# youngalip/clip-lora-match

Hardware: AMD Instinct MI355X
Metric: image+text embeds/sec & cosine top-k QPS, ViT-B/32+LoRA, 1/2/4/8 MI355X (higher is better)
Workload: dtype bf16 (vision) + fp16 (text); 1 GPU; ViT-B/32 + LoRA r=8 alpha=16 (q,k,v,out, both towers) encode + L2-normalise; per_gpu_batch=256, global_batch=256, seq_len=77, image_size=224, lora_mode=merged, parallelism=dp1

## Files before the change

clip-lora-match_amd/csrc/capi.cpp:

```cpp
#include <hip/hip_runtime.h>

#include <algorithm>
#include <cmath>
#include <map>
#include <mutex>
#include <tuple>
#include <cstdlib>
#include <cstring>
#include <string>
#include <unordered_map>
#include <vector>

#include "clm.h"
#include "kernels.hpp"

using namespace clm;

namespace {

thread_local std::string g_err;
int g_gemm_debug = getenv("CLM_GEMM_DEBUG") ? atoi(getenv("CLM_GEMM_DEBUG")) : 0;
int fail(int code, const std::string& msg) {
  g_err = msg;
  return code;
}
#define HIPCHK(x)                                                                              \
  do {                                                                                         \
    hipError_t e_ = (x);                                                                       \
    if (e_ != hipSuccess) return fail(CLM_E_HIP, std::string(#x) + ": " + hipGetErrorString(e_)); \
  } while (0)

struct DeviceGuard {
  int prev = -1;
  explicit DeviceGuard(int dev) {
    if (hipGetDevice(&prev) != hipSuccess) prev = -1;
    if (prev != dev) (void)hipSetDevice(dev);
  }
  ~DeviceGuard() {
    int cur = -1;
    if (prev >= 0 && hipGetDevice(&cur) == hipSuccess && cur != prev) (void)hipSetDevice(prev);
  }
};

bool is_device_ptr(const void* p) {
  if (!p) return false;
  hipPointerAttribute_t a;
  if (hipPointerGetAttributes(&a, p) != hipSuccess) {
    (void)hipGetLastError();
    return false;
  }
  return a.type == hipMemoryTypeDevice;
}

uint16_t host_f32_to_bf16(float f) {
  uint32_t u;
  std::memcpy(&u, &f, 4);
  if ((u & 0x7fffffffu) > 0x7f800000u) return (uint16_t)((u >> 16) | 0x40);
  u += 0x7fffu + ((u >> 16) & 1u);
  return (uint16_t)(u >> 16);
}
uint16_t host_f32_to_f16(float f) {
  _Float16 h = (_Float16)f;
  uint16_t r;
  std::memcpy(&r, &h, 2);
  return r;
}
float host_f16_to_f32(uint16_t v) {
  _Float16 h;
  std::memcpy(&h, &v, 2);
  return (float)h;
}
float host_bf16_to_f32(uint16_t v) {
  uint32_t u = (uint32_t)v << 16;
  float f;
  std::memcpy(&f, &u, 4);
  return f;
}

int64_t round_up(int64_t x, int64_t m) { return (x + m - 1) / m * m; }

struct HostTensor {
  std::vector<int64_t> shape;
  std::vector<float> data;
};

struct LayerW {
  float *ln1_g = nullptr, *ln1_b = nullptr, *ln2_g = nullptr, *ln2_b = nullptr;
  u16* w_qkv = nullptr; float* b_qkv = nullptr; int k_qkv = 0, kl_qkv = 0;
  u16* w_out = nullptr; float* b_out = nullptr; int k_out = 0, kl_out = 0;
  u16* w_fc1 = nullptr; float* b_fc1 = nullptr; int k_fc1 = 0, kl_fc1 = 0;
  u16* w_fc2 = nullptr; float* b_fc2 = nullptr; int k_fc2 = 0, kl_fc2 = 0;
  u16* a_qkv = nullptr; int r_qkv = 0;
  u16* a_out = nullptr; int r_out = 0;
  u16* a_fc1 = nullptr; int r_fc1 = 0;
  u16* a_fc2 = nullptr; int r_fc2 = 0;
};

struct Tower {
  bool vision = false;
  bool q_log2e = false;
  int d = 0, L = 0, H = 0, mlp = 0;
  std::vector<LayerW> layers;
  float *projT = nullptr, *fin_g = nullptr, *fin_b = nullptr;
  u16* patch_w = nullptr; int kp = 0;
  float *cls = nullptr, *pos = nullptr, *pre_g = nullptr, *pre_b = nullptr, *lut = nullptr;
  float *tok = nullptr, *tpos = nullptr;
  int64_t maxM = 0;
  float* h = nullptr;
  u16 *X = nullptr, *QKV = nullptr, *O = nullptr, *Hm = nullptr, *P = nullptr;
  float* pooled = nullptr;
  float* hc = nullptr;
  u16* Oc = nullptr;
  int *vl_lens = nullptr, *vl_offs = nullptr, *vl_rowmap = nullptr, *vl_tiles = nullptr, *vl_counts = nullptr;
  int64_t ldx = 0, ldo = 0, ldm = 0;
};

constexpr int RPAD = 64;
constexpr int LORA_GRANULE = 32;

}

struct clm_ctx {
  int dev = 0;
  clm_model_desc desc{};
  bool finalized = false;
  bool lora_enabled = true;
  std::unordered_map<std::string, HostTensor> host;
  std::vector<void*> allocs;
  Tower vis, txt;
  void* stage_in = nullptr; size_t stage_in_bytes = 0;
  void* stage_out = nullptr; size_t stage_out_bytes = 0;
  int32_t* ids_dev = nullptr;
  static constexpr int MAX_SPLIT = 4;
  hipStream_t ps[2 * MAX_SPLIT] = {};
  hipEvent_t pev[2 * MAX_SPLIT] = {};
  hipEvent_t ev_fork = nullptr, ev_done = nullptr;
  typedef std::tuple<const void*, int, int, const void*, int, int, void*, void*, int, int, int> PairKey;
  std::map<PairKey, hipGraphExec_t> graphs;
  int last_pair_path = -1;
  bool prof = false;
  std::vector<hipEvent_t> ev_pool;
  size_t ev_used = 0;
  struct Rec { int cat; double work; size_t e0, e1; };
  std::vector<Rec> recs;

  bool bf16(bool vision) const {
    return desc.compute_dtype == CLM_BF16 || (vision && desc.compute_dtype == CLM_COMPUTE_MIXED);
  }

  template <typename T>
  int dalloc(T** p, size_t count) {
    void* q = nullptr;
    if (count == 0) count = 1;
    if (hipMalloc(&q, count * sizeof(T)) != hipSuccess) {
      (void)hipGetLastError();
      return fail(CLM_E_OOM, "hipMalloc of " + std::to_string(count * sizeof(T)) + " bytes failed");
    }
    allocs.push_back(q);
    *p = (T*)q;
    return CLM_OK;
  }
  void drop_graphs() {
    for (auto& kv : graphs) (void)hipGraphExecDestroy(kv.second);
    graphs.clear();
  }
  void free_all() {
    drop_graphs();
    for (void* p : allocs) (void)hipFree(p);
    allocs.clear();
    if (stage_in) (void)hipFree(stage_in);
    if (stage_out) (void)hipFree(stage_out);
    stage_in = stage_out = nullptr;
    stage_in_bytes = stage_out_bytes = 0;
    vis = Tower();
    txt = Tower();
    ids_dev = nullptr;
  }
};

struct clm_index {
  int dev = 0;
  int64_t cap = 0, n = 0, dim = 0, offset = 0;
  u16* rows = nullptr;
  float* inv = nullptr;
  float* rows32 = nullptr;
  void* ws = nullptr; size_t ws_bytes = 0;
  void* ws2 = nullptr; size_t ws2_bytes = 0;
  void* ws3 = nullptr; size_t ws3_bytes = 0;
  void* ws4 = nullptr; size_t ws4_bytes = 0;
  u16* samp = nullptr; float* samp_inv = nullptr; int64_t samp_S = 0, samp_n = -1, samp_cap = 0;
  unsigned* inv_keys = nullptr; int64_t inv_keys_n = -1;
  int64_t search_stats[11] = {0, 0, 0, 0, 0, 0, 0, 0, 0, 0, 0};
};

namespace {

const HostTensor* find(const clm_ctx* c, const std::string& n) {
  auto it = c->host.find(n);
  return it == c->host.end() ? nullptr : &it->second;
}

int need(const clm_ctx* c, const std::string& n, int64_t numel, const HostTensor** out) {
  const HostTensor* t = find(c, n);
  if (!t) return fail(CLM_E_MISSING, "missing tensor '" + n + "'");
  if ((int64_t)t->data.size() != numel)
    return fail(CLM_E_ARG, "tensor '" + n + "' has " + std::to_string(t->data.size()) + " elements, expected " +
                               std::to_string(numel));
  *out = t;
  return CLM_OK;
}

int upload_f32(clm_ctx* c, const std::vector<float>& v, float** dst) {
  int r = c->dalloc(dst, v.size());
  if (r) return r;
  HIPCHK(hipMemcpy(*dst, v.data(), v.size() * sizeof(float), hipMemcpyHostToDevice));
  return CLM_OK;
}

int upload_16(clm_ctx* c, const std::vector<float>& v, u16** dst, bool bf) {
  std::vector<u16> h(v.size());
  if (bf)
    for (size_t i = 0; i < v.size(); ++i) h[i] = host_f32_to_bf16(v[i]);
  else
    for (size_t i = 0; i < v.size(); ++i) h[i] = host_f32_to_f16(v[i]);
  int r = c->dalloc(dst, h.size());
  if (r) return r;
  HIPCHK(hipMemcpy(*dst, h.data(), h.size() * sizeof(u16), hipMemcpyHostToDevice));
  return CLM_OK;
}

int upload_lora_a(clm_ctx* c, const std::vector<float>& A, int r_ext, int in, u16** dst, bool bf) {
  std::vector<float> pad((size_t)RPAD * in, 0.f);
  std::copy(A.begin(), A.begin() + (size_t)r_ext * in, pad.begin());
  return upload_16(c, pad, dst, bf);
}

int get_f32(clm_ctx* c, const std::string& n, int64_t numel, float** dst) {
  const HostTensor* t;
  int r = need(c, n, numel, &t);
  if (r) return r;
  return upload_f32(c, t->data, dst);
}

struct LinearSpec {
  std::string path;
  int in, out;
  bool lora;
};

int build_fused(clm_ctx* c, const std::vector<LinearSpec>& specs, float q_scale, std::vector<float>& W,
                std::vector<float>& bias, int& K, std::vector<float>& A_stack, int& r_ext, int& K_log) {
  const clm_model_desc& d = c->desc;
  const bool unmerged = d.lora_mode == CLM_LORA_UNMERGED;
  const int in = specs[0].in;
  int total_out = 0;
  r_ext = 0;
  for (auto& s : specs) {
    total_out += s.out;
    if (s.lora) r_ext += d.lora_r;
  }
  K = (unmerged && r_ext > 0) ? in + RPAD : in;
  K_log = (unmerged && r_ext > 0) ? in + (r_ext + LORA_GRANULE - 1) / LORA_GRANULE * LORA_GRANULE : in;
  if (r_ext > RPAD) return fail(CLM_E_ARG, "LoRA rank too large for the K-extension (sum r > 64)");
  W.assign((size_t)total_out * K, 0.f);
  bias.assign(total_out, 0.f);
  A_stack.assign((size_t)r_ext * in, 0.f);
  const float scaling = d.lora_r > 0 ? d.lora_alpha / (float)d.lora_r : 0.f;
  int row0 = 0, roff = 0;
  for (size_t si = 0; si < specs.size(); ++si) {
    const LinearSpec& s = specs[si];
    const HostTensor *w, *b;
    int r = need(c, s.path + ".weight", (int64_t)s.out * s.in, &w);
    if (r) return r;
    r = need(c, s.path + ".bias", s.out, &b);
    if (r) return r;
    const float qs = si == 0 ? q_scale : 1.0f;
    for (int o = 0; o < s.out; ++o) {
      std::memcpy(&W[(size_t)(row0 + o) * K], &w->data[(size_t)o * s.in], s.in * sizeof(float));
      bias[row0 + o] = b->data[o];
    }
    if (s.lora) {
      const HostTensor *A, *B;
      const std::string base = "base_model.model." + s.path;
      r = need(c, base + ".lora_A.weight", (int64_t)d.lora_r * s.in, &A);
      if (r) return r;
      r = need(c, base + ".lora_B.weight", (int64_t)s.out * d.lora_r, &B);
      if (r) return r;
      if (!unmerged) {
        for (int o = 0; o < s.out; ++o) {
          float* wr = &W[(size_t)(row0 + o) * K];
          for (int j = 0; j < d.lora_r; ++j) {
            const float bj = scaling * B->data[(size_t)o * d.lora_r + j];
            const float* ar = &A->data[(size_t)j * s.in];
            for (int i = 0; i < s.in; ++i) wr[i] += bj * ar[i];
          }
        }
      } else {
        for (int o = 0; o < s.out; ++o)
          for (int j = 0; j < d.lora_r; ++j)
            W[(size_t)(row0 + o) * K + s.in + roff + j] = scaling * B->data[(size_t)o * d.lora_r + j];
        std::memcpy(&A_stack[(size_t)roff * in], A->data.data(), (size_t)d.lora_r * in * sizeof(float));
      }
      roff += d.lora_r;
    }
    if (qs != 1.0f) {
      for (int o = 0; o < s.out; ++o) {
        float* wr = &W[(size_t)(row0 + o) * K];
        for (int i = 0; i < K; ++i) wr[i] *= qs;
        bias[row0 + o] *= qs;
      }
    }
    row0 += s.out;
  }
  if (!unmerged) r_ext = 0;
  return CLM_OK;
}

int build_tower(clm_ctx* c, Tower& T, bool vision) {
  const clm_model_desc& d = c->desc;
  const clm_tower_desc& td = vision ? d.vision : d.text;
  T.vision = vision;
  T.d = td.hidden; T.L = td.layers; T.H = td.heads; T.mlp = td.mlp;
  if (T.d != T.H * 64) return fail(CLM_E_ARG, "head_dim must be 64");
  if (T.d % 128 || T.d > 1024 || T.mlp % 64) return fail(CLM_E_ARG, "hidden must be a multiple of 128 (<=1024), mlp of 64");
  const std::string pre = vision ? "vision_model" : "text_model";
  const bool lora_on = c->lora_enabled && d.lora_r > 0;
  const uint32_t tg = lora_on ? d.lora_targets : 0u;
  const bool unmerged = d.lora_mode == CLM_LORA_UNMERGED;
  const int Tseq = vision ? (d.image_size / d.patch) * (d.image_size / d.patch) + 1 : 0;
  T.q_log2e = vision && attention_folds_log2e(c->bf16(true), false, Tseq);
  const float qscale = T.q_log2e ? 0.125f * 1.4426950408889634f : 0.125f;
  int r;
  T.layers.resize(T.L);
  for (int l = 0; l < T.L; ++l) {
    LayerW& Lw = T.layers[l];
    const std::string p = pre + ".encoder.layers." + std::to_string(l);
    if ((r = get_f32(c, p + ".layer_norm1.weight", T.d, &Lw.ln1_g))) return r;
    if ((r = get_f32(c, p + ".layer_norm1.bias", T.d, &Lw.ln1_b))) return r;
    if ((r = get_f32(c, p + ".layer_norm2.weight", T.d, &Lw.ln2_g))) return r;
    if ((r = get_f32(c, p + ".layer_norm2.bias", T.d, &Lw.ln2_b))) return r;
    std::vector<float> W, b, A;
    int K, rext, KL;
    std::vector<LinearSpec> qkv = {{p + ".self_attn.q_proj", T.d, T.d, (tg & CLM_LORA_Q) != 0},
                                   {p + ".self_attn.k_proj", T.d, T.d, (tg & CLM_LORA_K) != 0},
                                   {p + ".self_attn.v_proj", T.d, T.d, (tg & CLM_LORA_V) != 0}};
    if ((r = build_fused(c, qkv, qscale, W, b, K, A, rext, KL))) return r;
    if ((r = upload_16(c, W, &Lw.w_qkv, c->bf16(vision))) || (r = upload_f32(c, b, &Lw.b_qkv))) return r;
    Lw.k_qkv = K; Lw.kl_qkv = KL; Lw.r_qkv = rext;
    if (unmerged && rext && (r = upload_lora_a(c, A, rext, T.d, &Lw.a_qkv, c->bf16(vision)))) return r;

    std::vector<LinearSpec> outp = {{p + ".self_attn.out_proj", T.d, T.d, (tg & CLM_LORA_OUT) != 0}};
    if ((r = build_fused(c, outp, 1.0f, W, b, K, A, rext, KL))) return r;
    if ((r = upload_16(c, W, &Lw.w_out, c->bf16(vision))) || (r = upload_f32(c, b, &Lw.b_out))) return r;
    Lw.k_out = K; Lw.kl_out = KL; Lw.r_out = rext;
    if (unmerged && rext && (r = upload_lora_a(c, A, rext, T.d, &Lw.a_out, c->bf16(vision)))) return r;

    std::vector<LinearSpec> fc1 = {{p + ".mlp.fc1", T.d, T.mlp, (tg & CLM_LORA_FC1) != 0}};
    if ((r = build_fused(c, fc1, 1.0f, W, b, K, A, rext, KL))) return r;
    if ((r = upload_16(c, W, &Lw.w_fc1, c->bf16(vision))) || (r = upload_f32(c, b, &Lw.b_fc1))) return r;
    Lw.k_fc1 = K; Lw.kl_fc1 = KL; Lw.r_fc1 = rext;
    if (unmerged && rext && (r = upload_lora_a(c, A, rext, T.d, &Lw.a_fc1, c->bf16(vision)))) return r;

    std::vector<LinearSpec> fc2 = {{p + ".mlp.fc2", T.mlp, T.d, (tg & CLM_LORA_FC2) != 0}};
    if ((r = build_fused(c, fc2, 1.0f, W, b, K, A, rext, KL))) return r;
    if ((r = upload_16(c, W, &Lw.w_fc2, c->bf16(vision))) || (r = upload_f32(c, b, &Lw.b_fc2))) return r;
    Lw.k_fc2 = K; Lw.kl_fc2 = KL; Lw.r_fc2 = rext;
    if (unmerged && rext && (r = upload_lora_a(c, A, rext, T.mlp, &Lw.a_fc2, c->bf16(vision)))) return r;
  }
  {
    const HostTensor* pw;
    const std::string pn = vision ? "visual_projection.weight" : "text_projection.weight";
    if ((r = need(c, pn, (int64_t)d.proj_dim * T.d, &pw))) return r;
    std::vector<float> pt((size_t)T.d * d.proj_dim);
    for (int j = 0; j < d.proj_dim; ++j)
      for (int i = 0; i < T.d; ++i) pt[(size_t)i * d.proj_dim + j] = pw->data[(size_t)j * T.d + i];
    if ((r = upload_f32(c, pt, &T.projT))) return r;
  }
  const int64_t B = d.max_batch;
  if (vision) {
    const int G = d.image_size / d.patch, Tn = G * G + 1;
    if ((r = get_f32(c, pre + ".post_layernorm.weight", T.d, &T.fin_g))) return r;
    if ((r = get_f32(c, pre + ".post_layernorm.bias", T.d, &T.fin_b))) return r;
    if ((r = get_f32(c, pre + ".pre_layrnorm.weight", T.d, &T.pre_g))) return r;
    if ((r = get_f32(c, pre + ".pre_layrnorm.bias", T.d, &T.pre_b))) return r;
    if ((r = get_f32(c, pre + ".embeddings.class_embedding", T.d, &T.cls))) return r;
    if ((r = get_f32(c, pre + ".embeddings.position_embedding.weight", (int64_t)Tn * T.d, &T.pos))) return r;
    const int kreal = d.channels * d.patch * d.patch;
    T.kp = (int)round_up(kreal, 64);
    const HostTensor* pw;
    if ((r = need(c, pre + ".embeddings.patch_embedding.weight", (int64_t)T.d * kreal, &pw))) return r;
    std::vector<float> wp((size_t)T.d * T.kp, 0.f);
    for (int o = 0; o < T.d; ++o) std::memcpy(&wp[(size_t)o * T.kp], &pw->data[(size_t)o * kreal], kreal * 4);
    if ((r = upload_16(c, wp, &T.patch_w, c->bf16(true)))) return r;
    std::vector<float> lut((size_t)d.channels * 256);
    for (int ch = 0; ch < d.channels; ++ch)
      for (int u = 0; u < 256; ++u) {
        const float x = (float)((double)u * (1.0 / 255.0));
        lut[(size_t)ch * 256 + u] = (x - d.mean[ch % 3]) / d.std[ch % 3];
      }
    if ((r = upload_f32(c, lut, &T.lut))) return r;
    T.maxM = B * Tn;
    if ((r = c->dalloc(&T.P, (size_t)B * G * G * T.kp))) return r;
  } else {
    if ((r = get_f32(c, pre + ".final_layer_norm.weight", T.d, &T.fin_g))) return r;
    if ((r = get_f32(c, pre + ".final_layer_norm.bias", T.d, &T.fin_b))) return r;
    if ((r = get_f32(c, pre + ".embeddings.token_embedding.weight", (int64_t)d.vocab * T.d, &T.tok))) return r;
    if ((r = get_f32(c, pre + ".embeddings.position_embedding.weight", (int64_t)d.max_pos * T.d, &T.tpos))) return r;
    T.maxM = B * d.max_pos;
  }
  T.ldx = T.d + RPAD;
  T.ldo = T.d + RPAD;
  T.ldm = T.mlp + RPAD;
  if ((r = c->dalloc(&T.h, (size_t)T.maxM * T.d))) return r;
  if ((r = c->dalloc(&T.X, (size_t)T.maxM * T.ldx))) return r;
  if ((r = c->dalloc(&T.QKV, (size_t)T.maxM * 3 * T.d))) return r;
  if ((r = c->dalloc(&T.O, (size_t)T.maxM * T.ldo))) return r;
  if ((r = c->dalloc(&T.Hm, (size_t)T.maxM * T.ldm))) return r;
  if ((r = c->dalloc(&T.pooled, (size_t)B * d.proj_dim))) return r;
  if ((r = c->dalloc(&T.hc, (size_t)B * T.d))) return r;
  if ((r = c->dalloc(&T.Oc, (size_t)B * T.ldo))) return r;
  if (!T.vision) {
    if ((r = c->dalloc(&T.vl_lens, (size_t)B))) return r;
    if ((r = c->dalloc(&T.vl_offs, (size_t)2 * B + 1))) return r;
    if ((r = c->dalloc(&T.vl_rowmap, (size_t)T.maxM))) return r;
    if ((r = c->dalloc(&T.vl_tiles, (size_t)B))) return r;
    if ((r = c->dalloc(&T.vl_counts, (size_t)2 * B))) return r;
  }
  return CLM_OK;
}

int ensure_stage(void** p, size_t* cap, size_t bytes) {
  if (*cap >= bytes) return CLM_OK;
  if (*p) (void)hipFree(*p);
  *p = nullptr;
  *cap = 0;
  if (hipMalloc(p, bytes) != hipSuccess) {
    (void)hipGetLastError();
    *p = nullptr;
    return fail(CLM_E_OOM, "staging allocation failed");
  }
  *cap = bytes;
  return CLM_OK;
}

struct ProfScope {
  clm_ctx* c; hipStream_t st; int cat; double work; size_t e0 = 0; bool on = false;
  ProfScope(clm_ctx* c_, hipStream_t st_, int cat_, double work_) : c(c_), st(st_), cat(cat_), work(work_) {
    if (!c->prof) return;
    if (c->ev_used + 2 > c->ev_pool.size()) {
      for (int i = 0; i < 256; ++i) {
        hipEvent_t e;
        if (hipEventCreate(&e) != hipSuccess) { (void)hipGetLastError(); return; }
        c->ev_pool.push_back(e);
      }
    }
    e0 = c->ev_used;
    c->ev_used += 2;
    on = hipEventRecord(c->ev_pool[e0], st) == hipSuccess;
  }
  ~ProfScope() {
    if (!on) return;
    if (hipEventRecord(c->ev_pool[e0 + 1], st) == hipSuccess) c->recs.push_back({cat, work, e0, e0 + 1});
  }
};
#define PROF(cat, work) ProfScope prof_scope_##__LINE__(c, st, cat, work)

#define KCHK(x)                                                                                   \
  do {                                                                                            \
    hipError_t e_ = (x);                                                                          \
    if (e_ != hipSuccess) return fail(CLM_E_HIP, std::string("kernel launch ") + #x + ": " + hipGetErrorString(e_)); \
  } while (0)

LnArgs ln_into_x(clm_ctx* c, Tower& T, int64_t M, const float* g, const float* b, float* h = nullptr) {
  LnArgs a{};
  if (!h) h = T.h;
  a.mode = 0; a.src = h; a.lds = T.d; a.hf = h; a.ldh = T.d;
  a.g1 = g; a.b1 = b; a.y = T.X; a.ldy = T.ldx;
  a.M = (int)M; a.d = T.d; a.eps = c->desc.ln_eps;
  return a;
}

hipError_t lora_down_gemm(bool bf, u16* X, int64_t ldx, int M, int K, const u16* A, const int* mdev,
                          hipStream_t st) {
  GemmArgs g{};
  g.A = X; g.lda = ldx; g.W = A; g.ldw = K; g.M = M; g.N = RPAD; g.K = K;
  g.out = X + K; g.ldo = ldx; g.m_dev = mdev;
  static const int cfg = getenv("CLM_LORA_DOWN_CFG") ? atoi(getenv("CLM_LORA_DOWN_CFG")) : GEMM_CFG_SKINNY;
  return gemm_cfg(bf, EPI_STORE, cfg, g, st);
}

bool prune_last_layer() {
  static int v = -1;
  if (v < 0) {
    const char* e = getenv("CLM_NO_PRUNE");
    v = (e && atoi(e)) ? 0 : 1;
  }
  return v == 1 && !(g_gemm_debug & 8);
}

bool text_varlen_enabled() {
  static int v = -1;
  if (v < 0) {
    const char* e = getenv("CLM_TEXT_VARLEN");
    v = (e && !atoi(e)) ? 0 : 1;
  }
  return v == 1 && !(g_gemm_debug & 32);
}

bool fused_attention(int T, int H, int d, int K) {
  static int v = -1;
  if (v < 0) {
    const char* e = getenv("CLM_FUSED_ATTN");
    v = (e && !atoi(e)) ? 0 : 1;
  }
  return v == 1 && !(g_gemm_debug & 16) && gemm_attn_supported(T, H, d, K);
}

struct LayerRun {
  Tower* T;
  int B, S;
  bool causal, vl, bf;
  const int32_t* ids;
  const int* mdev;
  double Mx, attn_pairs;
};

int make_run(clm_ctx* c, Tower& T, int B, int S, bool causal, const int32_t* ids, bool vl, hipStream_t st,
             LayerRun* r) {
  *r = LayerRun{&T, B, S, causal, vl, c->bf16(T.vision), ids, vl ? T.vl_counts : nullptr, (double)B * S,
                (double)B * S * S};
  if (vl && c->prof) {
    std::vector<int> lens(B);
    HIPCHK(hipMemcpyAsync(lens.data(), T.vl_lens, (size_t)B * 4, hipMemcpyDeviceToHost, st));
    HIPCHK(hipStreamSynchronize(st));
    r->Mx = r->attn_pairs = 0;
    for (int v : lens) { r->Mx += v; r->attn_pairs += (double)v * v; }
  }
  return CLM_OK;
}

double attn_flops(const LayerRun& R, int l) {
  const Tower& T = *R.T;
  return 2.0 * R.Mx * 3 * T.d * T.layers[l].kl_qkv + 4.0 * T.H * R.attn_pairs * 64;
}

int attn_step(clm_ctx* c, const LayerRun& R, int l, hipStream_t st) {
  Tower& T = *R.T;
  LayerW& Lw = T.layers[l];
  const bool bf = R.bf;
  GemmArgs g{};
  g.A = T.X; g.lda = T.ldx; g.M = R.B * R.S; g.N = 3 * T.d; g.K = Lw.kl_qkv; g.out = T.QKV; g.ldo = 3 * T.d;
  g.W = Lw.w_qkv; g.ldw = Lw.k_qkv; g.bias = Lw.b_qkv;
  if (R.vl) {
    PROF(CLM_PROF_GEMM, attn_flops(R, l));
    KCHK(gemm_attn_varlen(bf, R.causal, g.A, g.lda, g.W, g.ldw, g.bias, T.O, T.ldo, R.B, R.S, T.H, T.d, g.K,
                          T.vl_lens, T.vl_offs, T.vl_tiles, T.vl_counts, st));
  } else if (fused_attention(R.S, T.H, T.d, g.K)) {
    PROF(CLM_PROF_GEMM, attn_flops(R, l));
    KCHK(gemm_attn(bf, R.causal, g.A, g.lda, g.W, g.ldw, g.bias, T.O, T.ldo, R.B, R.S, T.H, T.d, g.K, st));
  } else {
    { PROF(CLM_PROF_GEMM, 2.0 * g.M * g.N * g.K); KCHK(gemm(bf, EPI_STORE, g, st)); }
    { PROF(CLM_PROF_ATTN, 4.0 * R.B * T.H * (double)R.S * R.S * 64);
      KCHK(attention(bf, R.causal, T.QKV, 3 * T.d, T.O, T.ldo, R.B, R.S, T.H, T.d, st, T.q_log2e)); }
  }
  return CLM_OK;
}

int pooled_resid(clm_ctx* c, const LayerRun& R, GemmArgs& g, hipStream_t st) {
  const int nk = g.K / 64;
  int slices = 1;
  for (int sl = nk / 4; sl >= 2; --sl)
    if (nk % sl == 0 && gemm_splitk_ws_bytes(1, g.N, sl) <= (size_t)R.S * 3 * R.T->d * 2) { slices = sl; break; }
  PROF(CLM_PROF_GEMM, 2.0 * g.M * g.N * g.K);
  if (slices > 1) KCHK(gemm_splitk_resid(R.bf, g, slices, (float*)R.T->QKV, st));
  else KCHK(gemm_cfg(R.bf, EPI_RESID, GEMM_CFG_SPLITK, g, st));
  return CLM_OK;
}

struct PostOps {
  GemmArgs out, fc1, fc2;
  LnArgs ln2, ln1;
  bool has_ln1;
  double rows;
};
PostOps post_ops(clm_ctx* c, const LayerRun& R, int l, int64_t M, float* h, u16* O, bool pooled) {
  Tower& T = *R.T;
  LayerW& Lw = T.layers[l];
  const int* mdev = pooled ? nullptr : R.mdev;
  PostOps p{};
  p.rows = pooled ? (double)M : R.Mx;
  GemmArgs& g = p.out;
  g.A = O; g.lda = T.ldo; g.W = Lw.w_out; g.ldw = Lw.k_out; g.M = (int)M; g.N = T.d; g.K = pooled ? Lw.k_out : Lw.kl_out;
  g.out = h; g.ldo = T.d; g.bias = Lw.b_out; g.m_dev = mdev;
  p.ln2 = ln_into_x(c, T, M, Lw.ln2_g, Lw.ln2_b, h);
  p.ln2.m_dev = mdev;
  GemmArgs& f = p.fc1;
  f.A = T.X; f.lda = T.ldx; f.M = (int)M; f.N = T.mlp; f.K = Lw.k_fc1; f.out = T.Hm; f.ldo = T.ldm;
  f.W = Lw.w_fc1; f.ldw = Lw.k_fc1; f.bias = Lw.b_fc1; f.m_dev = mdev;
  GemmArgs& f2 = p.fc2;
  f2.A = T.Hm; f2.lda = T.ldm; f2.W = Lw.w_fc2; f2.ldw = Lw.k_fc2; f2.M = (int)M; f2.N = T.d;
  f2.K = pooled ? Lw.k_fc2 : Lw.kl_fc2;
  f2.out = h; f2.ldo = T.d; f2.bias = Lw.b_fc2; f2.m_dev = mdev;
  p.has_ln1 = l + 1 < T.L;
  if (p.has_ln1) {
    LayerW& Ln = T.layers[l + 1];
    p.ln1 = ln_into_x(c, T, M, Ln.ln1_g, Ln.ln1_b);
    p.ln1.m_dev = mdev;
  }
  return p;
}

int post_attn_step(clm_ctx* c, const LayerRun& R, int l, bool* pooled_rows, hipStream_t st) {
  Tower& T = *R.T;
  LayerW& Lw = T.layers[l];
  const bool bf = R.bf;
  const bool pooled = prune_last_layer() && l + 1 == T.L;
  int64_t M = (int64_t)R.B * R.S;
  float* h = T.h;
  u16* O = T.O;
  if (pooled) {
    { PROF(CLM_PROF_OTHER, (double)R.B * T.d * 6.0);
      KCHK(gather_pooled(T.h, T.d, T.O, T.ldo, R.B, R.S, T.d, R.ids, c->desc.eos_token_id, T.hc, T.Oc, T.ldo, st,
                         R.vl ? T.vl_offs : nullptr)); }
    M = R.B;
    h = T.hc;
    O = T.Oc;
    *pooled_rows = true;
  }
  PostOps p = post_ops(c, R, l, M, h, O, pooled);
  const int* mdev = pooled ? nullptr : R.mdev;
  if (Lw.r_out) { PROF(CLM_PROF_GEMM, 2.0 * p.rows * RPAD * T.d);
    KCHK(lora_down_gemm(bf, O, T.ldo, (int)M, T.d, Lw.a_out, mdev, st)); }
  if (pooled) {
    int r = pooled_resid(c, R, p.out, st);
    if (r) return r;
  } else {
    PROF(CLM_PROF_GEMM, 2.0 * p.rows * p.out.N * p.out.K); KCHK(gemm(bf, EPI_RESID, p.out, st));
  }
  { PROF(CLM_PROF_LN, p.rows * T.d * 6.0); KCHK(layernorm(bf, p.ln2, st)); }
  if (Lw.r_fc1) { PROF(CLM_PROF_GEMM, 2.0 * p.rows * RPAD * T.d);
    KCHK(lora_down_gemm(bf, T.X, T.ldx, (int)M, T.d, Lw.a_fc1, mdev, st)); }
  { PROF(CLM_PROF_GEMM, 2.0 * p.rows * p.fc1.N * p.fc1.K);
    KCHK(pooled ? gemm_cfg(bf, EPI_GELU, GEMM_CFG_SPLITK, p.fc1, st) : gemm(bf, EPI_GELU, p.fc1, st)); }
  if (Lw.r_fc2) { PROF(CLM_PROF_GEMM, 2.0 * p.rows * RPAD * T.mlp);
    KCHK(lora_down_gemm(bf, T.Hm, T.ldm, (int)M, T.mlp, Lw.a_fc2, mdev, st)); }
  if (pooled) {
    int r = pooled_resid(c, R, p.fc2, st);
    if (r) return r;
  } else {
    PROF(CLM_PROF_GEMM, 2.0 * p.rows * p.fc2.N * p.fc2.K); KCHK(gemm(bf, EPI_RESID, p.fc2, st));
  }
  if (p.has_ln1) {
    { PROF(CLM_PROF_LN, p.rows * T.d * 6.0); KCHK(layernorm(bf, p.ln1, st)); }
    const LayerW& Ln = T.layers[l + 1];
    if (Ln.r_qkv) { PROF(CLM_PROF_GEMM, 2.0 * p.rows * RPAD * T.d);
      KCHK(lora_down_gemm(bf, T.X, T.ldx, (int)M, T.d, Ln.a_qkv, mdev, st)); }
  }
  return CLM_OK;
}

int run_layers(clm_ctx* c, Tower& T, int B, int S, bool causal, const int32_t* ids, bool* pooled_rows,
               hipStream_t st, bool vl = false) {
  *pooled_rows = false;
  LayerRun R;
  int r = make_run(c, T, B, S, causal, ids, vl, st, &R);
  for (int l = 0; !r && l < T.L; ++l) {
    r = attn_step(c, R, l, st);
    if (!r) r = post_attn_step(c, R, l, pooled_rows, st);
  }
  return r;
}

Tower ws_view(const Tower& T0, int b0, int rows, int patches, int proj_dim) {
  Tower T = T0;
  const int64_t r0 = (int64_t)b0 * rows;
  T.h += r0 * T.d; T.X += r0 * T.ldx; T.QKV += r0 * 3 * T.d; T.O += r0 * T.ldo; T.Hm += r0 * T.ldm;
  if (T.P) T.P += (int64_t)b0 * patches * T.kp;
  T.pooled += (int64_t)b0 * proj_dim;
  T.hc += (int64_t)b0 * T.d;
  T.Oc += (int64_t)b0 * T.ldo;
  if (T.vl_lens) {
    T.vl_lens += b0; T.vl_tiles += b0; T.vl_offs += 2 * b0; T.vl_counts += 2 * b0; T.vl_rowmap += r0;
  }
  return T;
}

int image_prologue(clm_ctx* c, Tower& T, const void* pix, int layout, int B, hipStream_t st) {
  const clm_model_desc& d = c->desc;
  const bool bf = c->bf16(T.vision);
  const int G = d.image_size / d.patch, Tn = G * G + 1;
  { PROF(CLM_PROF_OTHER, (double)B * G * G * T.kp * 2.0 + (double)B * d.image_size * d.image_size * d.channels);
    KCHK(patchify(bf, pix, layout, B, d.image_size, d.patch, d.channels, T.lut, T.P, T.kp, st)); }
  GemmArgs g{};
  g.A = T.P; g.lda = T.kp; g.W = T.patch_w; g.ldw = T.kp; g.M = B * G * G; g.N = T.d; g.K = T.kp;
  g.out = T.h; g.ldo = T.d; g.aux = T.pos; g.aux_ld = T.d; g.group = G * G;
  { PROF(CLM_PROF_GEMM, 2.0 * g.M * g.N * g.K); KCHK(gemm(bf, EPI_PATCH, g, st)); }
  { PROF(CLM_PROF_OTHER, (double)B * T.d * 4.0); KCHK(write_cls(T.h, T.d, B, Tn, T.d, T.cls, T.pos, st)); }
  LnArgs a = ln_into_x(c, T, (int64_t)B * Tn, T.pre_g, T.pre_b);
  a.g2 = T.layers[0].ln1_g; a.b2 = T.layers[0].ln1_b;
  { PROF(CLM_PROF_LN, (double)B * Tn * T.d * 10.0); KCHK(layernorm(bf, a, st)); }
  if (T.layers[0].r_qkv) { PROF(CLM_PROF_GEMM, 2.0 * B * Tn * RPAD * T.d);
    KCHK(lora_down_gemm(bf, T.X, T.ldx, B * Tn, T.d, T.layers[0].a_qkv, nullptr, st)); }
  return CLM_OK;
}

int image_epilogue(clm_ctx* c, Tower& T, int B, bool pooled_rows, void* out, int out_dtype, int normalize,
                   hipStream_t st) {
  const clm_model_desc& d = c->desc;
  const int G = d.image_size / d.patch, Tn = G * G + 1;
  PROF(CLM_PROF_OTHER, (double)B * (T.d * 4.0 + d.proj_dim * 4.0) + (double)T.d * d.proj_dim * 4.0);
  KCHK(pool_project(pooled_rows ? T.hc : T.h, T.d, B, pooled_rows ? 1 : Tn, T.d, nullptr, d.eos_token_id, T.fin_g,
                    T.fin_b, d.ln_eps, T.projT, d.proj_dim, T.pooled, out, out_dtype == CLM_F32 ? 0 : 1, normalize,
                    st));
  return CLM_OK;
}

int encode_image_chunk(clm_ctx* c, Tower& T, const void* pix, int layout, int B, void* out, int out_dtype,
                       int normalize, hipStream_t st) {
  const int G = c->desc.image_size / c->desc.patch;
  int r = image_prologue(c, T, pix, layout, B, st);
  bool pooled_rows = false;
  if (!r) r = run_layers(c, T, B, G * G + 1, false, nullptr, &pooled_rows, st);
  if (!r) r = image_epilogue(c, T, B, pooled_rows, out, out_dtype, normalize, st);
  return r;
}

int text_prologue(clm_ctx* c, Tower& T, const int32_t* ids_dev, int B, int L, bool* vl_out, hipStream_t st) {
  const clm_model_desc& d = c->desc;
  const bool bf = c->bf16(T.vision);
  LnArgs a{};
  a.mode = 1; a.ids = ids_dev; a.tok = T.tok; a.pos = T.tpos; a.L = L;
  a.hf = T.h; a.ldh = T.d; a.g1 = T.layers[0].ln1_g; a.b1 = T.layers[0].ln1_b;
  a.y = T.X; a.ldy = T.ldx; a.M = B * L; a.d = T.d; a.eps = d.ln_eps;
  bool vl = text_varlen_enabled() && T.vl_lens && B <= 4096 &&
            fused_attention(L, T.H, T.d, T.layers.empty() ? 0 : T.layers[0].k_qkv);
  if (vl) {
    { PROF(CLM_PROF_OTHER, (double)B * L * 8.0);
      KCHK(text_plan(ids_dev, B, L, d.eos_token_id, T.vl_lens, T.vl_offs, T.vl_rowmap, T.vl_tiles, T.vl_counts, st)); }
    a.m_dev = T.vl_counts;
    a.rowmap = T.vl_rowmap;
  }
  *vl_out = vl;
  { PROF(CLM_PROF_LN, (double)B * L * T.d * 14.0); KCHK(layernorm(bf, a, st)); }
  if (T.layers[0].r_qkv) { PROF(CLM_PROF_GEMM, 2.0 * B * L * RPAD * T.d);
    KCHK(lora_down_gemm(bf, T.X, T.ldx, B * L, T.d, T.layers[0].a_qkv, vl ? T.vl_counts : nullptr, st)); }
  return CLM_OK;
}

int text_epilogue(clm_ctx* c, Tower& T, const int32_t* ids_dev, int B, int L, bool vl, bool pooled_rows, void* out,
                  int out_dtype, int normalize, hipStream_t st) {
  const clm_model_desc& d = c->desc;
  PROF(CLM_PROF_OTHER, (double)B * (T.d * 4.0 + d.proj_dim * 4.0 + L * 4.0) + (double)T.d * d.proj_dim * 4.0);
  KCHK(pool_project(pooled_rows ? T.hc : T.h, T.d, B, pooled_rows ? 1 : L, T.d, pooled_rows ? nullptr : ids_dev,
                    d.eos_token_id, T.fin_g, T.fin_b, d.ln_eps, T.projT, d.proj_dim, T.pooled, out,
                    out_dtype == CLM_F32 ? 0 : 1, normalize, st, vl && !pooled_rows ? T.vl_offs : nullptr));
  return CLM_OK;
}

int encode_text_chunk(clm_ctx* c, Tower& T, const int32_t* ids_dev, int B, int L, void* out, int out_dtype,
                      int normalize, hipStream_t st) {
  bool vl = false, pooled_rows = false;
  int r = text_prologue(c, T, ids_dev, B, L, &vl, st);
  if (!r) r = run_layers(c, T, B, L, true, ids_dev, &pooled_rows, st, vl);
  if (!r) r = text_epilogue(c, T, ids_dev, B, L, vl, pooled_rows, out, out_dtype, normalize, st);
  return r;
}

size_t dtype_size(int dt) {
  switch (dt) {
    case CLM_F32: case CLM_I32: return 4;
    case CLM_F16: case CLM_BF16: return 2;
    case CLM_U8: return 1;
    case CLM_I64: return 8;
  }
  return 0;
}

}

extern "C" {

const char* clm_last_error(void) { return g_err.c_str(); }
const char* clm_version(void) { return "clm 0.1.0 gfx950"; }
int32_t clm_model_desc_size(void) { return (int32_t)sizeof(clm_model_desc); }

int clm_gemm(int hip_device, int dtype, int epilogue, int config, const void* A, int64_t lda, const void* W,
             int64_t ldw, int M, int N, int K, void* out, int64_t ldo, const float* bias, const float* rscale,
             const float* cscale, void* stream) {
  if (dtype != CLM_BF16 && dtype != CLM_F16) return fail(CLM_E_ARG, "dtype must be bf16 or f16");
  if (epilogue != EPI_STORE && epilogue != EPI_GELU && epilogue != EPI_RESID && epilogue != EPI_SCORE)
    return fail(CLM_E_ARG, "bad epilogue");
  if (config >= gemm_num_configs()) return fail(CLM_E_ARG, "bad config");
  const int64_t kr = (K + 63) / 64 * 64;
  if (M < 0 || N < 0 || K <= 0 || K % 32 || (K % 64 && (lda < kr || ldw < kr)))
    return fail(CLM_E_ARG, "bad shape (K % 64 == 0, or K % 64 == 32 with lda, ldw >= round_up(K, 64))");
  DeviceGuard g(hip_device);
  GemmArgs a{};
  a.A = (const u16*)A; a.lda = lda; a.W = (const u16*)W; a.ldw = ldw; a.M = M; a.N = N; a.K = K;
  a.out = out; a.ldo = ldo; a.bias = bias; a.rscale = rscale; a.cscale = cscale;
  a.debug = g_gemm_debug;
  hipError_t e = gemm_cfg(dtype == CLM_BF16, epilogue, config, a, (hipStream_t)stream);
  if (e != hipSuccess) return fail(CLM_E_HIP, std::string("gemm: ") + hipGetErrorString(e));
  return CLM_OK;
}

int clm_gemm_num_configs(void) { return gemm_num_configs(); }

int clm_gemm_scores16(int hip_device, int config, const void* A, int64_t lda, const void* W, int64_t ldw, int M,
                      int N, int K, const float* rscale, const float* cscale, void* out, int64_t ldo, int mode,
                      void* stream) {
  if (mode != 1 && mode != 2) return fail(CLM_E_ARG, "mode must be 1 (fp16 scores) or 2 (group maxima)");
  if (config >= gemm_num_configs()) return fail(CLM_E_ARG, "bad config");
  if (M < 0 || N < 0 || K <= 0 || K % 64) return fail(CLM_E_ARG, "bad shape (K % 64 == 0)");
  if (mode == 2 && (config != 1 || N % 256 || ldo < N / 4 || ldo % 8))
    return fail(CLM_E_ARG, "group maxima: config 1, N % 256 == 0, ldo >= N / 4, ldo % 8 == 0");
  if (mode == 1 && ldo < N) return fail(CLM_E_ARG, "ldo < N");
  DeviceGuard g(hip_device);
  GemmArgs a{};
  a.A = (const u16*)A; a.lda = lda; a.W = (const u16*)W; a.ldw = ldw; a.M = M; a.N = N; a.K = K;
  a.out = out; a.ldo = ldo; a.rscale = rscale; a.cscale = cscale; a.out16 = mode;
  hipError_t e = gemm_cfg(false, EPI_SCORE, config, a, (hipStream_t)stream);
  if (e != hipSuccess) return fail(CLM_E_HIP, std::string("gemm: ") + hipGetErrorString(e));
  return CLM_OK;
}

void clm_debug_set(int flags) { g_gemm_debug = flags; }

int clm_attention_ex(int hip_device, int dtype, int flags, const void* qkv, void* out, int64_t ldo, int B, int T,
                     int H, void* stream) {
  if (dtype != CLM_BF16 && dtype != CLM_F16) return fail(CLM_E_ARG, "dtype must be bf16 or f16");
  if (B < 0 || T < 0 || H <= 0) return fail(CLM_E_ARG, "bad shape");
  DeviceGuard g(hip_device);
  if (flags & ~(CLM_ATTN_CAUSAL | CLM_ATTN_Q_LOG2E)) return fail(CLM_E_ARG, "unknown attention flags");
  const bool bf = dtype == CLM_BF16, cz = (flags & CLM_ATTN_CAUSAL) != 0, l2e = (flags & CLM_ATTN_Q_LOG2E) != 0;
  if (l2e && !attention_folds_log2e(bf, cz, T))
    return fail(CLM_E_ARG, "CLM_ATTN_Q_LOG2E: the kernel for this dtype / mask / T takes q without log2(e)");
  hipError_t e = attention(bf, cz, (const u16*)qkv, 3LL * H * 64, (u16*)out, ldo, B, T, H, H * 64,
                           (hipStream_t)stream, l2e);
  if (e != hipSuccess) return fail(CLM_E_HIP, std::string("attention: ") + hipGetErrorString(e));
  return CLM_OK;
}

int clm_attention(int hip_device, int dtype, int causal, const void* qkv, void* out, int64_t ldo, int B, int T,
                  int H, void* stream) {
  return clm_attention_ex(hip_device, dtype, causal ? CLM_ATTN_CAUSAL : 0, qkv, out, ldo, B, T, H, stream);
}

int clm_layernorm(int hip_device, int dtype, const float* src, int64_t lds, int64_t M, int d, const float* gamma,
                  const float* beta, float eps, void* y, int64_t ldy, void* stream) {
  if (dtype != CLM_BF16 && dtype != CLM_F16) return fail(CLM_E_ARG, "dtype must be bf16 or f16");
  if (M < 0 || M > 0x7FFFFFFF || d <= 0 || d % 128 || d > 1024 || lds < d || ldy < d || (lds % 4) || (ldy % 4))
    return fail(CLM_E_ARG, "bad shape");
  if (M == 0) return CLM_OK;
  DeviceGuard g(hip_device);
  LnArgs a{};
  a.mode = 0; a.src = src; a.lds = lds; a.hf = nullptr; a.ldh = 0;
  a.g1 = gamma; a.b1 = beta; a.y = (u16*)y; a.ldy = ldy; a.M = (int)M; a.d = d; a.eps = eps;
  hipError_t e = layernorm(dtype == CLM_BF16, a, (hipStream_t)stream);
  if (e != hipSuccess) return fail(CLM_E_HIP, std::string("layernorm: ") + hipGetErrorString(e));
  return CLM_OK;
}

int clm_prof_enable(clm_ctx* ctx, int enable) {
  if (!ctx) return fail(CLM_E_ARG, "null ctx");
  DeviceGuard g(ctx->dev);
  (void)hipDeviceSynchronize();
  ctx->prof = enable != 0;
  ctx->recs.clear();
  ctx->ev_used = 0;
  return CLM_OK;
}

int clm_prof_read(clm_ctx* ctx, int category, double* ms, double* work, int64_t* launches) {
  if (!ctx || category < 0 || category >= CLM_PROF_NCAT) return fail(CLM_E_ARG, "bad argument");
  DeviceGuard g(ctx->dev);
  double t = 0, w = 0;
  int64_t n = 0;
  for (auto& r : ctx->recs) {
    if (r.cat != category) continue;
    HIPCHK(hipEventSynchronize(ctx->ev_pool[r.e1]));
    float m = 0.f;
    HIPCHK(hipEventElapsedTime(&m, ctx->ev_pool[r.e0], ctx->ev_pool[r.e1]));
    t += m; w += r.work; ++n;
  }
  if (ms) *ms = t;
  if (work) *work = w;
  if (launches) *launches = n;
  return CLM_OK;
}

int clm_ctx_create(int hip_device, const clm_model_desc* desc, clm_ctx** out) {
  if (!desc || !out) return fail(CLM_E_ARG, "null argument");
  int ndev = 0;
  if (hipGetDeviceCount(&ndev) != hipSuccess || ndev <= 0) {
    (void)hipGetLastError();
    return fail(CLM_E_HIP, "no HIP device available");
  }
  if (hip_device < 0 || hip_device >= ndev) return fail(CLM_E_ARG, "bad device index");
  if (desc->compute_dtype != CLM_BF16 && desc->compute_dtype != CLM_F16 && desc->compute_dtype != CLM_COMPUTE_MIXED)
    return fail(CLM_E_ARG, "compute_dtype must be CLM_BF16, CLM_F16 or CLM_COMPUTE_MIXED");
  if (desc->max_batch <= 0 || desc->patch <= 0 || desc->image_size % desc->patch)
    return fail(CLM_E_ARG, "bad max_batch / patch / image_size");
  if (desc->max_pos > 77 * 4 || desc->proj_dim > 1024) return fail(CLM_E_ARG, "bad max_pos / proj_dim");
  if (desc->lora_r < 0 || desc->lora_r > 64) return fail(CLM_E_ARG, "lora_r must be in [0, 64]");
  clm_ctx* c = new clm_ctx();
  c->dev = hip_device;
  c->desc = *desc;
  *out = c;
  return CLM_OK;
}

int clm_ctx_destroy(clm_ctx* ctx) {
  if (!ctx) return CLM_OK;
  DeviceGuard g(ctx->dev);
  (void)hipDeviceSynchronize();
  ctx->free_all();
  for (hipEvent_t e : ctx->ev_pool) (void)hipEventDestroy(e);
  for (hipEvent_t e : {ctx->ev_fork, ctx->ev_done})
    if (e) (void)hipEventDestroy(e);
  for (int i = 0; i < 2 * clm_ctx::MAX_SPLIT; ++i) {
    if (ctx->pev[i]) (void)hipEventDestroy(ctx->pev[i]);
    if (ctx->ps[i]) (void)hipStreamDestroy(ctx->ps[i]);
  }
  delete ctx;
  return CLM_OK;
}

int clm_load_tensor(clm_ctx* ctx, const char* name, const void* host_ptr, int dtype, const int64_t* shape,
                    int ndim) {
  if (!ctx || !name || (!host_ptr && ndim > 0) || ndim < 0 || ndim > 8) return fail(CLM_E_ARG, "bad argument");
  int64_t n = 1;
  HostTensor t;
  for (int i = 0; i < ndim; ++i) {
    if (shape[i] < 0) return fail(CLM_E_ARG, "negative dim");
    n *= shape[i];
    t.shape.push_back(shape[i]);
  }
  t.data.resize(n);
  if (dtype == CLM_F32) {
    std::memcpy(t.data.data(), host_ptr, n * sizeof(float));
  } else if (dtype == CLM_F16) {
    const uint16_t* p = (const uint16_t*)host_ptr;
    for (int64_t i = 0; i < n; ++i) t.data[i] = host_f16_to_f32(p[i]);
  } else if (dtype == CLM_BF16) {
    const uint16_t* p = (const uint16_t*)host_ptr;
    for (int64_t i = 0; i < n; ++i) t.data[i] = host_bf16_to_f32(p[i]);
  } else {
    return fail(CLM_E_ARG, "tensor dtype must be f32/f16/bf16");
  }
  ctx->host[name] = std::move(t);
  ctx->finalized = false;
  return CLM_OK;
}

int clm_finalize(clm_ctx* ctx) {
  if (!ctx) return fail(CLM_E_ARG, "null ctx");
  DeviceGuard g(ctx->dev);
  (void)hipDeviceSynchronize();
  ctx->free_all();
  ctx->finalized = false;
  int r = build_tower(ctx, ctx->vis, true);
  if (!r) r = build_tower(ctx, ctx->txt, false);
  if (!r) r = ctx->dalloc(&ctx->ids_dev, (size_t)ctx->desc.max_batch * ctx->desc.max_pos);
  if (r) {
    ctx->free_all();
    return r;
  }
  ctx->finalized = true;
  return CLM_OK;
}

int clm_set_lora(clm_ctx* ctx, int r, float alpha, uint32_t targets) {
  if (!ctx) return fail(CLM_E_ARG, "null ctx");
  if (r < 0 || r > 64) return fail(CLM_E_ARG, "lora_r must be in [0, 64]");
  if (targets & ~(uint32_t)(CLM_LORA_Q | CLM_LORA_K | CLM_LORA_V | CLM_LORA_OUT | CLM_LORA_FC1 | CLM_LORA_FC2))
    return fail(CLM_E_ARG, "unknown LoRA target bits");
  ctx->desc.lora_r = r;
  ctx->desc.lora_alpha = alpha;
  ctx->desc.lora_targets = r > 0 ? targets : 0u;
  ctx->finalized = false;
  return CLM_OK;
}

// ... 1556 lines not shown
```

clip-lora-match_amd/csrc/clm_common.hpp:

```cpp
#pragma once
#include <hip/hip_runtime.h>
#include <stdint.h>

typedef uint16_t u16;
typedef __bf16 bf16x8 __attribute__((ext_vector_type(8)));
typedef _Float16 f16x8 __attribute__((ext_vector_type(8)));
typedef float f32x4 __attribute__((ext_vector_type(4)));
typedef uint32_t u32x4 __attribute__((ext_vector_type(4)));
typedef uint32_t u32x2 __attribute__((ext_vector_type(2)));

constexpr uint32_t BUF_OOB = 0x80000000u;
__device__ __forceinline__ __amdgpu_buffer_rsrc_t buf_rsrc(const void* base, int num_records = 0x7FFFFFF0) {
  const uint64_t b = (uint64_t)base;
  const uint32_t lo = __builtin_amdgcn_readfirstlane((uint32_t)b);
  const uint32_t hi = __builtin_amdgcn_readfirstlane((uint32_t)(b >> 32));
  return __builtin_amdgcn_make_buffer_rsrc((void*)(((uint64_t)hi << 32) | lo), 0, num_records, 0x00020000);
}

namespace clm {

constexpr int WAVE = 64;

__device__ __forceinline__ float bf16_to_f32(u16 v) { return __uint_as_float(((uint32_t)v) << 16); }
__device__ __forceinline__ float f16_to_f32(u16 v) { return (float)__builtin_bit_cast(_Float16, v); }
__device__ __forceinline__ u16 f32_to_bf16(float f) { return __builtin_bit_cast(u16, (__bf16)f); }
__device__ __forceinline__ u16 f32_to_f16(float f) { return __builtin_bit_cast(u16, (_Float16)f); }

template <bool BF> __device__ __forceinline__ float to_f32(u16 v) { return BF ? bf16_to_f32(v) : f16_to_f32(v); }
template <bool BF> __device__ __forceinline__ u16 from_f32(float f) { return BF ? f32_to_bf16(f) : f32_to_f16(f); }

typedef __bf16 bf16x2_t __attribute__((ext_vector_type(2)));
typedef _Float16 f16x2_t __attribute__((ext_vector_type(2)));
typedef float f32x2_t __attribute__((ext_vector_type(2)));
template <bool BF> __device__ __forceinline__ uint32_t pack2(float a, float b) {
#ifdef CLM_PACK_SCALAR
  return (uint32_t)from_f32<BF>(a) | ((uint32_t)from_f32<BF>(b) << 16);
#else
  if constexpr (BF)
    return __builtin_bit_cast(uint32_t, __builtin_convertvector(f32x2_t{a, b}, bf16x2_t));
  else
    return __builtin_bit_cast(uint32_t, __builtin_convertvector(f32x2_t{a, b}, f16x2_t));
#endif
}

template <bool BF>
__device__ __forceinline__ f32x4 mfma16(const u32x4& a, const u32x4& b, f32x4 c) {
  if constexpr (BF)
    return __builtin_amdgcn_mfma_f32_16x16x32_bf16(__builtin_bit_cast(bf16x8, a),
                                                   __builtin_bit_cast(bf16x8, b), c, 0, 0, 0);
  else
    return __builtin_amdgcn_mfma_f32_16x16x32_f16(__builtin_bit_cast(f16x8, a),
                                                  __builtin_bit_cast(f16x8, b), c, 0, 0, 0);
}

template <int CTRL> __device__ __forceinline__ float dpp_f(float v) {
  return __builtin_bit_cast(float, __builtin_amdgcn_update_dpp(0, __builtin_bit_cast(int, v), CTRL, 0xF, 0xF, false));
}
template <bool MAX> __device__ __forceinline__ float op2(float a, float b) { return MAX ? fmaxf(a, b) : a + b; }
template <bool MAX> __device__ __forceinline__ float row16_reduce(float v) {
  v = op2<MAX>(v, dpp_f<0xB1>(v));
  v = op2<MAX>(v, dpp_f<0x4E>(v));
  v = op2<MAX>(v, dpp_f<0x141>(v));
  v = op2<MAX>(v, dpp_f<0x140>(v));
  return v;
}
template <bool MAX> __device__ __forceinline__ float cross_rows_reduce(float v) {
  const auto r = __builtin_amdgcn_permlane16_swap(__float_as_uint(v), __float_as_uint(v), false, false);
  v = op2<MAX>(__uint_as_float(r[0]), __uint_as_float(r[1]));
  const auto t = __builtin_amdgcn_permlane32_swap(__float_as_uint(v), __float_as_uint(v), false, false);
  return op2<MAX>(__uint_as_float(t[0]), __uint_as_float(t[1]));
}
template <bool MAX> __device__ __forceinline__ float wave_reduce(float v) {
  return cross_rows_reduce<MAX>(row16_reduce<MAX>(v));
}
__device__ __forceinline__ float wave_sum(float v) { return wave_reduce<false>(v); }
__device__ __forceinline__ float wave_max(float v) { return wave_reduce<true>(v); }
__device__ __forceinline__ float group16_sum(float v) { return row16_reduce<false>(v); }
__device__ __forceinline__ float group16_max(float v) { return row16_reduce<true>(v); }

__device__ __forceinline__ uint32_t f16_down(float v) {
  const _Float16 h = (_Float16)v;
  uint32_t b = __builtin_bit_cast(uint16_t, h);
  if ((float)h > v) b = b == 0u ? 0x8001u : (b & 0x8000u) ? b + 1u : b - 1u;
  return b;
}

__device__ __forceinline__ float quick_gelu(float x) {
  const float t = __builtin_amdgcn_exp2f(-2.4554669595930157f * x);
  return x * __builtin_amdgcn_rcpf(1.0f + t);
}

__device__ __forceinline__ int swz(int row, int chunk) { return chunk ^ ((row >> 1) & 7); }

__device__ __forceinline__ int xcd_remap(int bid, int nwg) {
  const int q = nwg / 8, r = nwg % 8, x = bid % 8;
  return (x < r ? x * (q + 1) : r * (q + 1) + (x - r) * q) + bid / 8;
}

}
```

clip-lora-match_amd/csrc/k_gemm.hip:

```cpp
#include <algorithm>
#include <cstdlib>
#include <vector>

#include "gemm_common.hpp"

namespace clm {

namespace {
using namespace gemm_detail;
template <bool BF, int EPI, int BM, int BN, int WM, int WN, int STAGES>
__device__ __forceinline__ void gemm_body(const GemmArgs& ga, int bid, int G) {
  using C = Cfg<BM, BN, WM, WN, STAGES>;
  GemmArgs g = ga;
  if (g.m_dev) g.M = __builtin_amdgcn_readfirstlane(*g.m_dev);
  extern __shared__ __attribute__((aligned(16))) uint8_t smem[];
  const int tid = threadIdx.x, lane = tid & 63;
  const int wid = __builtin_amdgcn_readfirstlane(tid >> 6);
  const int ntn = (g.N + BN - 1) / BN, ntm = (g.M + BM - 1) / BM;
  const int ks = g.ksplit > 1 ? g.ksplit : 1;
  const int ntiles = ntn * ntm * ks;
  const TileWalk tw = tile_walk(ntiles, bid, G);
  if (tw.count <= 0) return;
  const int n_my = tw.count;
  const int nk = (g.K + BK - 1) / BK / ks;
  const bool half_last = (g.K % BK) != 0;
  const int S = n_my * nk;

  auto coords = [&](int i, int& m0, int& n0, int& k0) {
    int t = tw.first + i * tw.stride;
    k0 = 0;
    if (ks > 1) {
      k0 = (t % ks) * nk * BK;
      t /= ks;
    }
    int tm, tn;
    if (g.m_fastest) {
      tm = t % ntm;
      tn = t / ntm;
    } else {
      const int group = t / (GM * ntn);
      const int first_m = group * GM;
      const int gsz = min(GM, ntm - first_m);
      const int r = t - group * GM * ntn;
      tm = first_m + r % gsz;
      tn = r / gsz;
    }
    m0 = tm * BM;
    n0 = tn * BN;
  };

  const int r8 = lane >> 3, pc = lane & 7;
  const u16* a_src[C::LA];
  const u16* w_src[C::LB];
  auto point = [&](int i) {
    int m0, n0, k0;
    coords(i, m0, n0, k0);
#pragma unroll
    for (int j = 0; j < C::LA; ++j) {
      const int row = (wid * C::LA + j) * 8 + r8;
      a_src[j] = g.A + (int64_t)min(m0 + row, g.M - 1) * g.lda + k0 + (pc ^ ((row >> 1) & 7)) * 8;
    }
#pragma unroll
    for (int j = 0; j < C::LB; ++j) {
      const int row = (wid * C::LB + j) * 8 + r8;
      w_src[j] = g.W + (int64_t)min(n0 + row, g.N - 1) * g.ldw + k0 + (pc ^ ((row >> 1) & 7)) * 8;
    }
  };
  int ld_i = 0, ld_kt = 0;
  point(0);
  auto stage_next = [&](int buf) {
    uint8_t* base = smem + buf * C::STAGE_BYTES;
#pragma unroll
    for (int j = 0; j < C::LA; ++j)
      __builtin_amdgcn_global_load_lds((const void*)(a_src[j] + ld_kt * BK),
                                       (void*)(base + (wid * C::LA + j) * 1024), 16, 0, 0);
#pragma unroll
    for (int j = 0; j < C::LB; ++j)
      __builtin_amdgcn_global_load_lds((const void*)(w_src[j] + ld_kt * BK),
                                       (void*)(base + BM * 128 + (wid * C::LB + j) * 1024), 16, 0, 0);
    if (++ld_kt == nk) {
      ld_kt = 0;
      if (++ld_i < n_my) point(ld_i);
    }
  };

  const int wm = wid / WN, wn = wid % WN;
  f32x4 acc[C::TM][C::TN];
#pragma unroll
  for (int i = 0; i < C::TM; ++i)
#pragma unroll
    for (int j = 0; j < C::TN; ++j) acc[i][j] = f32x4{0.f, 0.f, 0.f, 0.f};

#pragma unroll
  for (int s = 0; s < STAGES - 1; ++s)
    if (s < S) stage_next(s);

  constexpr int E0 = epi_min_stores<EPI, C::TM, C::TN>();
  constexpr int E = E0 + C::L * (STAGES - 2) > 63 ? 63 - C::L * (STAGES - 2) : E0;
  const bool vec_epi = (g.N % 4) == 0 && (g.ldo % 4) == 0 && !(g.debug & 1);
  int c_i = 0, c_kt = 0, m0, n0, k0;
  coords(0, m0, n0, k0);
  int since_end = STAGES;
  constexpr int PB = (EPI == EPI_RESID && STAGES == 2 && C::TN == 6) ? 1 : 0;
  constexpr bool PRE = PB > 0;
  constexpr int XP = PB * C::TN;
  u32x4 hpre[PRE ? PB : 1][C::TN];
  const bool pre_on = PRE && ks == 1 && nk >= 2 && vec_epi;
  bool hp_pending = false;
  for (int s = 0; s < S; ++s) {
    const bool more = s + STAGES - 2 < S;
    ++since_end;
    const bool pe = vec_epi && since_end <= STAGES - 1;
    if (PRE && hp_pending) {
      wait_vmcnt<XP>();
      hp_pending = false;
    } else if (more) {
      if (pe) wait_vmcnt<C::L * (STAGES - 2) + E>();
      else wait_vmcnt<C::L * (STAGES - 2)>();
    } else {
      if (pe) wait_vmcnt<E>();
      else wait_vmcnt<0>();
    }
    lds_barrier();
    if (s + STAGES - 1 < S) stage_next((s + STAGES - 1) % STAGES);
    if constexpr (PRE) {
      if (pre_on && c_kt == nk - 2) {
        resid_prefetch<BM, BN, WM, WN, PRE ? PB : 1>(g, m0, n0, wm, wn, lane, hpre);
        hp_pending = true;
      }
    }
    const uint8_t* sa = smem + (s % STAGES) * C::STAGE_BYTES;
    const uint8_t* sb = sa + BM * 128;
#pragma unroll
    for (int kk = 0; kk < 2; ++kk) {
      if (kk == 1 && half_last && c_kt == nk - 1) break;
      const int c = kk * 4 + (lane >> 4);
      u32x4 af[C::TM], bw[C::TN];
#pragma unroll
      for (int mb = 0; mb < C::TM; ++mb) {
        const int row = wm * (BM / WM) + mb * 16 + (lane & 15);
        af[mb] = *(const u32x4*)(sa + row * 128 + swz(row, c) * 16);
      }
#pragma unroll
      for (int nb = 0; nb < C::TN; ++nb) {
        const int row = wn * (BN / WN) + nb * 16 + (lane & 15);
        bw[nb] = *(const u32x4*)(sb + row * 128 + swz(row, c) * 16);
      }
#pragma unroll
      for (int mb = 0; mb < C::TM; ++mb)
#pragma unroll
        for (int nb = 0; nb < C::TN; ++nb) acc[mb][nb] = mfma16<BF>(bw[nb], af[mb], acc[mb][nb]);
    }
    if (++c_kt == nk) {
      since_end = 0;
      if (g.debug & 1) {
#pragma unroll
        for (int mb = 0; mb < C::TM; ++mb)
#pragma unroll
          for (int nb = 0; nb < C::TN; ++nb) asm volatile("" ::"v"(acc[mb][nb]));
      } else {
        if constexpr (PRE) {
          if (pre_on) epilogue<BF, EPI, BM, BN, WM, WN, STAGES, PB>(g, acc, m0, n0, wm, wn, lane, 0, hpre);
          else epilogue<BF, EPI, BM, BN, WM, WN, STAGES>(g, acc, m0, n0, wm, wn, lane, 0);
        } else {
          epilogue<BF, EPI, BM, BN, WM, WN, STAGES>(g, acc, m0, n0, wm, wn, lane,
                                                    ks > 1 ? (int64_t)(k0 / (nk * BK)) * g.split_stride : 0);
        }
      }
#pragma unroll
      for (int i = 0; i < C::TM; ++i)
#pragma unroll
        for (int j = 0; j < C::TN; ++j) acc[i][j] = f32x4{0.f, 0.f, 0.f, 0.f};
      c_kt = 0;
      if (++c_i < n_my) coords(c_i, m0, n0, k0);
    }
  }
}

template <bool BF, int EPI, int BM, int BN, int WM, int WN, int STAGES>
__global__ __launch_bounds__(WM * WN * 64, (Cfg<BM, BN, WM, WN, STAGES>::WAVES_PER_EU)) void gemm_kernel(GemmArgs ga) {
  gemm_body<BF, EPI, BM, BN, WM, WN, STAGES>(ga, blockIdx.x, gridDim.x);
}

template <bool BF, int EPI, int BM, int BN, int WM, int WN, int STAGES>
hipError_t launch_cfg(const GemmArgs& g, hipStream_t s) {
  using C = Cfg<BM, BN, WM, WN, STAGES>;
  auto kern = gemm_kernel<BF, EPI, BM, BN, WM, WN, STAGES>;
  static unsigned dev_done = 0;
  int dev = 0;
  (void)hipGetDevice(&dev);
  if (!(__atomic_load_n(&dev_done, __ATOMIC_ACQUIRE) & (1u << (dev & 31)))) {
    hipError_t e = hipFuncSetAttribute((const void*)kern, hipFuncAttributeMaxDynamicSharedMemorySize, C::LDS);
    if (e != hipSuccess) return e;
    __atomic_fetch_or(&dev_done, 1u << (dev & 31), __ATOMIC_RELEASE);
  }
  static int slots[32] = {};
  int& sl = slots[dev & 31];
  if (sl == 0) {
    int per_cu = 0, cus = 0;
    if (hipOccupancyMaxActiveBlocksPerMultiprocessor(&per_cu, kern, C::NT, C::LDS) != hipSuccess || per_cu < 1) per_cu = 1;
    if (hipDeviceGetAttribute(&cus, hipDeviceAttributeMultiprocessorCount, dev) != hipSuccess || cus < 1) cus = 256;
    (void)hipGetLastError();
    sl = per_cu * cus;
  }
  const int tiles = ((g.N + BN - 1) / BN) * ((g.M + BM - 1) / BM) * (g.ksplit > 1 ? g.ksplit : 1);
  const int nwg = (g.debug & 4) ? tiles : std::min(tiles, sl);
  kern<<<dim3(nwg), dim3(C::NT), C::LDS, s>>>(g);
  return hipGetLastError();
}

template <bool BF, int EPI>
hipError_t launch_id(int id, const GemmArgs& g, hipStream_t s) {
  switch (id) {
    case 0: return launch_cfg<BF, EPI, 128, 128, 2, 2, 2>(g, s);
    case 1: return launch_cfg<BF, EPI, 256, 256, 4, 2, 2>(g, s);
    case 2: return launch_cfg<BF, EPI, 128, 64, 4, 1, 3>(g, s);
    case 3: return launch_cfg<BF, EPI, 128, 192, 2, 2, 2>(g, s);
    case 4: return launch_cfg<BF, EPI, 192, 128, 2, 2, 2>(g, s);
    case 5: return launch_cfg<BF, EPI, 256, 128, 4, 2, 2>(g, s);
    case 6: return launch_cfg<BF, EPI, 128, 256, 2, 4, 2>(g, s);
    case 7: return launch_cfg<BF, EPI, 160, 128, 2, 2, 2>(g, s);
    case 8: case 9: case 10: case 11: return gemm2_launch(BF, EPI, id, g, s);
    case 12: return launch_cfg<BF, EPI, 64, 64, 4, 1, 3>(g, s);
    case 13: case 14: return gemm4_launch(BF, EPI, id, g, s);
    default: return hipErrorInvalidValue;
  }
}

constexpr int NCFG = 15;
static_assert(GEMM_CFG_SKINNY == 12, "config 12 is the 64 x 64 tile");
static_assert(GEMM_CFG_SPLITK == 2, "config 2 is the 128 x 64 tile");

struct CfgModel { int id, bm, bn, wg_per_cu; double eff; };
constexpr CfgModel MODELS_G2[] = {
  {8, 256, 192, 1, 2.569}, {9, 256, 128, 1, 2.349}, {10, 192, 256, 1, 2.521}, {11, 128, 256, 1, 2.340}};
constexpr CfgModel MODELS[] = {
  {0, 128, 128, 2, 0.975}, {1, 256, 256, 1, 1.18}, {3, 128, 192, 2, 0.955}, {4, 192, 128, 2, 0.955},
  {5, 256, 128, 1, 1.025}, {6, 128, 256, 1, 1.056}, {7, 160, 128, 2, 0.93}};
thread_local bool g_concurrent = false;
bool env_concurrent() {
  static const int v = getenv("CLM_GEMM_CONCURRENT") ? atoi(getenv("CLM_GEMM_CONCURRENT")) : 0;
  return v != 0;
}
template <int NM>
int pick_from(const CfgModel (&models)[NM], int M, int N) {
  const int skip = (g_concurrent || env_concurrent()) ? 7 : -1;
  int best = models[0].id;
  double best_cost = 1e300;
  for (const CfgModel& c : models) {
    if (c.id == skip) continue;
    const int64_t tiles = (int64_t)((M + c.bm - 1) / c.bm) * ((N + c.bn - 1) / c.bn);
    const int64_t slots = 256LL * c.wg_per_cu;
    const int64_t rounds = (tiles + slots - 1) / slots;
    const double cost = rounds * (double)c.bm * c.bn * c.wg_per_cu / c.eff;
    if (cost < best_cost * 0.999) { best_cost = cost; best = c.id; }
  }
  return best;
}
int pick_config(int epi, int M, int N) {
  static int forced = -2;
  if (forced == -2) {
    const char* e = getenv("CLM_GEMM_CFG");
    forced = e ? atoi(e) : -1;
  }
  if (epi == EPI_RANK) return (forced == 1 || (forced >= 8 && forced <= 11)) ? forced : pick_from(MODELS_G2, M, N);
  if (forced >= 0 && forced < NCFG) return forced;
  if (epi == EPI_FILTER) return pick_from(MODELS_G2, M, N);
  static const int g4_store = getenv("CLM_G4_STORE") ? atoi(getenv("CLM_G4_STORE")) : 1;
  if (epi == EPI_STORE && g4_store && (int64_t)((M + 255) / 256) * ((N + 255) / 256) >= 4 * 256) return 13;
  if (epi != EPI_GELU) return pick_from(MODELS, M, N);
  if ((int64_t)((M + 255) / 256) * ((N + 255) / 256) >= 4 * 256) return 1;
  return pick_from(MODELS_G2, M, N);
}

template <bool BF>
hipError_t dispatch(int epi, int id, const GemmArgs& g, hipStream_t s) {
  switch (epi) {
    case EPI_STORE: return launch_id<BF, EPI_STORE>(id, g, s);
    case EPI_GELU: return launch_id<BF, EPI_GELU>(id, g, s);
    case EPI_RESID: return launch_id<BF, EPI_RESID>(id, g, s);
    case EPI_PATCH: return launch_id<BF, EPI_PATCH>(id, g, s);
    case EPI_SCORE: return launch_id<BF, EPI_SCORE>(id, g, s);
    case EPI_FILTER: return launch_id<BF, EPI_FILTER>(id, g, s);
    case EPI_RANK:
      if constexpr (!BF) {
        if (id == 1) return launch_cfg<false, EPI_RANK, 256, 256, 4, 2, 2>(g, s);
        if (id >= 8 && id <= 11) return gemm2_launch(false, EPI_RANK, id, g, s);
      }
      return hipErrorInvalidValue;
    default: return hipErrorInvalidValue;
  }
}
}

int gemm_num_configs() { return NCFG; }

hipError_t gemm_cfg(bool bf16, int epi, int config, const GemmArgs& g, hipStream_t s) {
  if (g.M <= 0 || g.N <= 0) return hipSuccess;
  if (g.K <= 0 || (g.K % 32) != 0 || (g.lda % 8) != 0 || (g.ldw % 8) != 0) return hipErrorInvalidValue;
  int id = config >= 0 ? config : pick_config(epi, g.M, g.N);
  if (g.K % BK) {
    if (g.ksplit > 1) return hipErrorInvalidValue;
    if (id >= 8 && id <= 11) {
      if (config >= 0) return hipErrorInvalidValue;
      id = pick_from(MODELS, g.M, g.N);
    }
  }
  if (id >= 13 && !gemm4_supports(epi, g)) {
    if (config >= 0) return hipErrorInvalidValue;
    id = pick_from(MODELS, g.M, g.N);
  }
  return bf16 ? dispatch<true>(epi, id, g, s) : dispatch<false>(epi, id, g, s);
}

hipError_t gemm(bool bf16, int epi, const GemmArgs& g, hipStream_t s) {
  if (g.ksplit > 1) return hipErrorInvalidValue;
  return gemm_cfg(bf16, epi, -1, g, s);
}

namespace {
__global__ __launch_bounds__(256) void splitk_resid_kernel(const float* ws, int slices, int M, int N, const float* bias,
                                                          float* out, int64_t ldo) {
  const int n4 = N / 4;
  const int64_t i = (int64_t)blockIdx.x * 256 + threadIdx.x;
  if (i >= (int64_t)M * n4) return;
  const int m = (int)(i / n4), n = (int)(i - (int64_t)m * n4) * 4;
  const int64_t stride = (int64_t)M * N;
  float4 acc = *(const float4*)(ws + (int64_t)m * N + n);
  for (int s = 1; s < slices; ++s) {
    const float4 p = *(const float4*)(ws + s * stride + (int64_t)m * N + n);
    acc.x += p.x; acc.y += p.y; acc.z += p.z; acc.w += p.w;
  }
  const float4 b = bias ? *(const float4*)(bias + n) : make_float4(0.f, 0.f, 0.f, 0.f);
  float4* o = (float4*)(out + (int64_t)m * ldo + n);
  float4 h = *o;
  h.x = h.x + (acc.x + b.x); h.y = h.y + (acc.y + b.y); h.z = h.z + (acc.z + b.z); h.w = h.w + (acc.w + b.w);
  *o = h;
}
}

hipError_t gemm_splitk_resid(bool bf16, const GemmArgs& g, int slices, float* ws, hipStream_t s) {
  if (g.M <= 0 || g.N <= 0) return hipSuccess;
  if (slices < 1 || g.K <= 0 || g.K % (BK * slices) || (g.N % 4) || (g.ldo % 4) || !ws) return hipErrorInvalidValue;
  GemmArgs p = g;
  p.out = ws; p.ldo = g.N; p.bias = nullptr; p.rscale = nullptr; p.cscale = nullptr;
  p.ksplit = slices; p.split_stride = (int64_t)g.M * g.N;
  hipError_t e = gemm_cfg(bf16, EPI_SCORE, GEMM_CFG_SPLITK, p, s);
  if (e != hipSuccess) return e;
  const int64_t n = (int64_t)g.M * (g.N / 4);
  splitk_resid_kernel<<<(unsigned)((n + 255) / 256), 256, 0, s>>>(ws, slices, g.M, g.N, g.bias, (float*)g.out, g.ldo);
  return hipGetLastError();
}

void gemm_set_concurrent(bool on) { g_concurrent = on; }

}
```

clip-lora-match_amd/csrc/k_gemm_attn.hip:

```cpp
#include <algorithm>

#include "gemm_common.hpp"

namespace clm {

namespace {
using namespace gemm_detail;

constexpr int FA_BM = 256, FA_BN = 192, FA_WM = 4, FA_WN = 2, FA_NW = 8;
constexpr int FA_TM = FA_BM / FA_WM / 16, FA_TN = FA_BN / FA_WN / 16;
constexpr int FA_LA = FA_BM / 8 / FA_NW, FA_LB = FA_BN / 8 / FA_NW;
constexpr int FA_STAGE = (FA_BM + FA_BN) * 128;
constexpr int FA_LDS = 2 * FA_STAGE;
constexpr int FA_SEC = FA_BM * 128;
static_assert(3 * FA_SEC <= FA_LDS, "q/k/v staging must fit in the ring's LDS");
static_assert(FA_BM % (8 * FA_NW) == 0 && FA_BN % (8 * FA_NW) == 0, "rows split evenly over waves");

__device__ __forceinline__ int swz_s(int row, int chunk) { return chunk ^ (row & 7); }

__device__ __forceinline__ u32x4 v_frag_rows(const uint8_t* sec, int kbase, int nb, int lane) {
  typedef short s16x4 __attribute__((ext_vector_type(4)));
  const int g = lane >> 4, i = lane & 15, q = i >> 2, p = i & 3;
  const int chunk = nb * 2 + (p >> 1);
  const int ka = min(kbase + g * 4 + q, FA_BM - 1), kb = min(kbase + 16 + g * 4 + q, FA_BM - 1);
  const uint8_t* pa = sec + ka * 128 + (swz_s(ka, chunk) << 4) + (p & 1) * 8;
  const uint8_t* pb = sec + kb * 128 + (swz_s(kb, chunk) << 4) + (p & 1) * 8;
  const s16x4 ra = __builtin_amdgcn_ds_read_tr16_b64_v4i16((__attribute__((address_space(3))) s16x4*)pa);
  const s16x4 rb = __builtin_amdgcn_ds_read_tr16_b64_v4i16((__attribute__((address_space(3))) s16x4*)pb);
  const u32x2 x = __builtin_bit_cast(u32x2, ra), y = __builtin_bit_cast(u32x2, rb);
  return u32x4{x.x, x.y, y.x, y.y};
}

struct FaArgs {
  const u16* X; int64_t ldx;
  const u16* W; int64_t ldw;
  const float* bias;
  u16* out; int64_t ldo;
  int B, T, H, d, K, G;
  const int* lens; const int* offs; const int* tiles; const int* counts;
};

template <bool BF, bool CAUSAL, bool VL>
__device__ __forceinline__ void gemm_attn_body(const FaArgs& a, int bid, int nwg) {
  extern __shared__ __attribute__((aligned(16))) uint8_t smem[];
  const int tid = threadIdx.x, lane = tid & 63, g = lane >> 4;
  const int wid = __builtin_amdgcn_readfirstlane(tid >> 6);
  int t, s0, nseq;
  int64_t m0, M;
  if constexpr (VL) {
    const int live = __builtin_amdgcn_readfirstlane(a.counts[1]) * a.H;
    if (bid >= live) return;
    t = xcd_remap(bid, live);
    const int tw = __builtin_amdgcn_readfirstlane(a.tiles[t / a.H]);
    s0 = tw & 0xFFFF;
    nseq = tw >> 16;
    m0 = __builtin_amdgcn_readfirstlane(a.offs[s0]);
    M = __builtin_amdgcn_readfirstlane(a.counts[0]);
  } else {
    t = xcd_remap(bid, nwg);
    s0 = (t / a.H) * a.G;
    nseq = min(a.G, a.B - s0);
    m0 = (int64_t)s0 * a.T;
    M = (int64_t)a.B * a.T;
  }
  const int h = t % a.H;
  const int nk = (a.K + BK - 1) / BK;
  const bool half_last = (a.K % BK) != 0;

  const int r8 = lane >> 3, pc = lane & 7;
  const u16* a_src[FA_LA];
  const u16* w_src[FA_LB];
#pragma unroll
  for (int j = 0; j < FA_LA; ++j) {
    const int row = (wid * FA_LA + j) * 8 + r8;
    a_src[j] = a.X + min(m0 + row, M - 1) * a.ldx + (pc ^ ((row >> 1) & 7)) * 8;
  }
#pragma unroll
  for (int j = 0; j < FA_LB; ++j) {
    const int row = (wid * FA_LB + j) * 8 + r8;
    const int64_t wrow = (int64_t)(row >> 6) * a.d + h * 64 + (row & 63);
    w_src[j] = a.W + wrow * a.ldw + (pc ^ ((row >> 1) & 7)) * 8;
  }
  auto stage = [&](int kt, int buf) {
    uint8_t* base = smem + buf * FA_STAGE;
#pragma unroll
    for (int j = 0; j < FA_LA; ++j)
      __builtin_amdgcn_global_load_lds((const void*)(a_src[j] + kt * BK), (void*)(base + (wid * FA_LA + j) * 1024),
                                       16, 0, 0);
#pragma unroll
    for (int j = 0; j < FA_LB; ++j)
      __builtin_amdgcn_global_load_lds((const void*)(w_src[j] + kt * BK),
                                       (void*)(base + FA_BM * 128 + (wid * FA_LB + j) * 1024), 16, 0, 0);
  };

  const int wm = wid / FA_WN, wn = wid % FA_WN;
  float4 bv[FA_TN];
#pragma unroll
  for (int nb = 0; nb < FA_TN; ++nb) {
    const int col = wn * (FA_BN / FA_WN) + nb * 16 + 4 * g;
    bv[nb] = a.bias ? *(const float4*)(a.bias + (col >> 6) * a.d + h * 64 + (col & 63)) : make_float4(0.f, 0.f, 0.f, 0.f);
  }
  f32x4 acc[FA_TM][FA_TN];
#pragma unroll
  for (int i = 0; i < FA_TM; ++i)
#pragma unroll
    for (int j = 0; j < FA_TN; ++j) acc[i][j] = f32x4{0.f, 0.f, 0.f, 0.f};

  stage(0, 0);
  for (int s = 0; s < nk; ++s) {
    wait_vmcnt<0>();
    lds_barrier();
    if (s + 1 < nk) stage(s + 1, (s + 1) & 1);
    const uint8_t* sa = smem + (s & 1) * FA_STAGE;
    const uint8_t* sb = sa + FA_BM * 128;
#pragma unroll
    for (int kk = 0; kk < 2; ++kk) {
      if (kk == 1 && half_last && s == nk - 1) break;
      const int c = kk * 4 + g;
      u32x4 af[FA_TM], bw[FA_TN];
#pragma unroll
      for (int mb = 0; mb < FA_TM; ++mb) {
        const int row = wm * (FA_BM / FA_WM) + mb * 16 + (lane & 15);
        af[mb] = *(const u32x4*)(sa + row * 128 + swz(row, c) * 16);
      }
#pragma unroll
      for (int nb = 0; nb < FA_TN; ++nb) {
        const int row = wn * (FA_BN / FA_WN) + nb * 16 + (lane & 15);
        bw[nb] = *(const u32x4*)(sb + row * 128 + swz(row, c) * 16);
      }
#pragma unroll
      for (int mb = 0; mb < FA_TM; ++mb)
#pragma unroll
        for (int nb = 0; nb < FA_TN; ++nb) acc[mb][nb] = mfma16<BF>(bw[nb], af[mb], acc[mb][nb]);
    }
  }

  lds_barrier();
  static_assert(FA_TN % 2 == 0, "column blocks are swapped in pairs");
#pragma unroll
  for (int mb = 0; mb < FA_TM; ++mb) {
    const int row = wm * (FA_BM / FA_WM) + mb * 16 + (lane & 15);
#pragma unroll
    for (int nb = 0; nb < FA_TN; nb += 2) {
      const u32x2 p0{pack2<BF>(acc[mb][nb][0] + bv[nb].x, acc[mb][nb][1] + bv[nb].y),
                     pack2<BF>(acc[mb][nb][2] + bv[nb].z, acc[mb][nb][3] + bv[nb].w)};
      const u32x2 p1{pack2<BF>(acc[mb][nb + 1][0] + bv[nb + 1].x, acc[mb][nb + 1][1] + bv[nb + 1].y),
                     pack2<BF>(acc[mb][nb + 1][2] + bv[nb + 1].z, acc[mb][nb + 1][3] + bv[nb + 1].w)};
      const auto rx = __builtin_amdgcn_permlane16_swap(p0.x, p1.x, false, false);
      const auto ry = __builtin_amdgcn_permlane16_swap(p0.y, p1.y, false, false);
      const int col = wn * (FA_BN / FA_WN) + (nb + (g & 1)) * 16 + (g >> 1) * 8;
      const int dim = col & 63;
      *(u32x4*)(smem + (col >> 6) * FA_SEC + row * 128 + (swz_s(row, dim >> 3) << 4)) = u32x4{rx[0], ry[0], rx[1], ry[1]};
    }
  }
  lds_barrier();

  constexpr float L2E = 1.4426950408889634f;
  const uint8_t* sQ = smem;
  const uint8_t* sK = smem + FA_SEC;
  const uint8_t* sV = smem + 2 * FA_SEC;
  int u = 0, i = 0, qb = 0, nqb = 0, seq_t = 0, seq_r0 = 0;
  auto load_seq = [&]() {
    if constexpr (VL) {
      seq_t = a.lens[s0 + i];
      seq_r0 = a.offs[s0 + i] - (int)m0;
    } else {
      seq_t = a.T;
      seq_r0 = i * a.T;
    }
    nqb = (seq_t + 15) / 16;
    qb = 0;
  };
  if (nseq > 0) load_seq();
  for (; i < nseq; ++u) {
    const int q0 = qb * 16, T = seq_t, r0 = seq_r0;
    const bool mine = (u % FA_NW) == wid;
    if (++qb == nqb && ++i < nseq) load_seq();
    if (!mine) continue;
    const int ntiles = (T + 63) / 64;
    const int qi = q0 + (lane & 15);
    u32x4 qa[2];
    {
      const int qrow = r0 + min(qi, T - 1);
#pragma unroll
      for (int kk = 0; kk < 2; ++kk) qa[kk] = *(const u32x4*)(sQ + qrow * 128 + swz_s(qrow, kk * 4 + g) * 16);
    }
    const int nkt = CAUSAL ? min((q0 + 15) / 64 + 1, ntiles) : ntiles;
    f32x4 sc[2][4];
    float tmax = -INFINITY;
#pragma unroll
    for (int kt = 0; kt < 2; ++kt) {
      if (kt >= nkt) break;
#pragma unroll
      for (int nb = 0; nb < 4; ++nb) {
        sc[kt][nb] = f32x4{0.f, 0.f, 0.f, 0.f};
        const int krow = min(r0 + kt * 64 + nb * 16 + (lane & 15), FA_BM - 1);
#pragma unroll
        for (int kk = 0; kk < 2; ++kk) {
          const int c = kk * 4 + g;
          sc[kt][nb] = mfma16<BF>(*(const u32x4*)(sK + krow * 128 + swz_s(krow, c) * 16), qa[kk], sc[kt][nb]);
        }
#pragma unroll
        for (int j = 0; j < 4; ++j) {
          const int kj = kt * 64 + nb * 16 + 4 * g + j;
          if (!(kj < T && (!CAUSAL || kj <= qi))) sc[kt][nb][j] = -INFINITY;
          tmax = fmaxf(tmax, sc[kt][nb][j]);
        }
      }
    }
    tmax = cross_rows_reduce<true>(tmax);
    const float m2 = tmax * L2E;
    float rs = 0.f;
    f32x4 o[4];
#pragma unroll
    for (int nb = 0; nb < 4; ++nb) o[nb] = f32x4{0.f, 0.f, 0.f, 0.f};
#pragma unroll
    for (int kt = 0; kt < 2; ++kt) {
      if (kt >= nkt) break;
      u32x4 pb[2];
#pragma unroll
      for (int nb = 0; nb < 4; ++nb)
#pragma unroll
        for (int j = 0; j < 4; ++j) {
          const float p = __builtin_amdgcn_exp2f(fmaf(sc[kt][nb][j], L2E, -m2));
          sc[kt][nb][j] = p;
          rs += p;
        }
#pragma unroll
      for (int kk = 0; kk < 2; ++kk) {
        const f32x4 lo = sc[kt][2 * kk], hi = sc[kt][2 * kk + 1];
        pb[kk] = u32x4{pack2<BF>(lo[0], lo[1]), pack2<BF>(lo[2], lo[3]), pack2<BF>(hi[0], hi[1]),
                       pack2<BF>(hi[2], hi[3])};
      }
#pragma unroll
      for (int kk = 0; kk < 2; ++kk)
#pragma unroll
        for (int nb = 0; nb < 4; ++nb)
          o[nb] = mfma16<BF>(v_frag_rows(sV, r0 + kt * 64 + kk * 32, nb, lane), pb[kk], o[nb]);
    }
    rs = cross_rows_reduce<false>(rs);
    if (qi < T) {
      const float inv = 1.0f / rs;
      u16* op = a.out + (m0 + r0 + qi) * a.ldo + h * 64 + 4 * g;
#pragma unroll
      for (int nb = 0; nb < 4; ++nb)
        *(u32x2*)(op + nb * 16) = u32x2{pack2<BF>(o[nb][0] * inv, o[nb][1] * inv), pack2<BF>(o[nb][2] * inv, o[nb][3] * inv)};
    }
  }
}

template <bool BF, bool CAUSAL, bool VL>
__global__ __launch_bounds__(FA_NW * 64, 2) void gemm_attn_kernel(FaArgs a) {
  gemm_attn_body<BF, CAUSAL, VL>(a, blockIdx.x, gridDim.x);
}

template <bool BF, bool CAUSAL, bool VL>
hipError_t launch(const FaArgs& a, int tiles, hipStream_t s) {
  auto kern = gemm_attn_kernel<BF, CAUSAL, VL>;
  static unsigned dev_done = 0;
  int dev = 0;
  (void)hipGetDevice(&dev);
  if (!(__atomic_load_n(&dev_done, __ATOMIC_ACQUIRE) & (1u << (dev & 31)))) {
    hipError_t e = hipFuncSetAttribute((const void*)kern, hipFuncAttributeMaxDynamicSharedMemorySize, FA_LDS);
    if (e != hipSuccess) return e;
    __atomic_fetch_or(&dev_done, 1u << (dev & 31), __ATOMIC_RELEASE);
  }
  kern<<<dim3(tiles), dim3(FA_NW * 64), FA_LDS, s>>>(a);
  return hipGetLastError();
}
}

bool gemm_attn_supported(int T, int H, int d, int K) {
  return T >= 1 && T <= 128 && d == H * 64 && K > 0 && K % 32 == 0;
}

namespace {
bool fixed_args(const AttnProblem& p, FaArgs& a, int& grid) {
  if (!gemm_attn_supported(p.T, p.H, p.d, p.K) || (p.ldx % 8) || (p.ldw % 8) || (p.ldo % 4) || p.ldx < p.K ||
      p.ldw < p.K || p.ldo < p.d)
    return false;
  a = FaArgs{};
  a.X = p.X; a.ldx = p.ldx; a.W = p.W; a.ldw = p.ldw; a.bias = p.bias; a.out = p.out; a.ldo = p.ldo;
  a.B = p.B; a.T = p.T; a.H = p.H; a.d = p.d; a.K = p.K; a.G = FA_BM / p.T;
  const int64_t tiles = (int64_t)((p.B + a.G - 1) / a.G) * p.H;
  if (tiles > 0x7FFFFFFF) return false;
  grid = (int)tiles;
  return true;
}
bool varlen_args(const AttnProblem& p, FaArgs& a, int& grid) {
  if (!gemm_attn_supported(p.T, p.H, p.d, p.K) || p.B > 0xFFFF || (p.ldx % 8) || (p.ldw % 8) || (p.ldo % 4) ||
      p.ldx < p.K || p.ldw < p.K || p.ldo < p.d || !p.lens || !p.offs || !p.tiles || !p.counts)
    return false;
  a = FaArgs{};
  a.X = p.X; a.ldx = p.ldx; a.W = p.W; a.ldw = p.ldw; a.bias = p.bias; a.out = p.out; a.ldo = p.ldo;
  a.B = p.B; a.T = p.T; a.H = p.H; a.d = p.d; a.K = p.K; a.G = 0;
  a.lens = p.lens; a.offs = p.offs; a.tiles = p.tiles; a.counts = p.counts;
  const int64_t max_tiles = std::min<int64_t>(p.B, ((int64_t)p.B * p.T + (256 - p.T)) / (257 - p.T) + 1);
  const int64_t g = max_tiles * p.H;
  if (g > 0x7FFFFFFF) return false;
  grid = (int)g;
  return true;
}
}

hipError_t gemm_attn(bool bf16, bool causal, const u16* X, int64_t ldx, const u16* W, int64_t ldw, const float* bias,
                     u16* out, int64_t ldo, int B, int T, int H, int d, int K, hipStream_t s) {
  if (B <= 0) return hipSuccess;
  AttnProblem p{X, ldx, W, ldw, bias, out, ldo, B, T, H, d, K, nullptr, nullptr, nullptr, nullptr};
  FaArgs a;
  int tiles;
  if (!fixed_args(p, a, tiles)) return hipErrorInvalidValue;
  if (bf16) return causal ? launch<true, true, false>(a, tiles, s) : launch<true, false, false>(a, tiles, s);
  return causal ? launch<false, true, false>(a, tiles, s) : launch<false, false, false>(a, tiles, s);
}

hipError_t gemm_attn_varlen(bool bf16, bool causal, const u16* X, int64_t ldx, const u16* W, int64_t ldw,
                            const float* bias, u16* out, int64_t ldo, int B, int L, int H, int d, int K,
                            const int* lens, const int* offs, const int* tiles, const int* counts, hipStream_t s) {
  if (B <= 0) return hipSuccess;
  AttnProblem p{X, ldx, W, ldw, bias, out, ldo, B, L, H, d, K, lens, offs, tiles, counts};
  FaArgs a;
  int grid;
  if (!varlen_args(p, a, grid)) return hipErrorInvalidValue;
  if (bf16) return causal ? launch<true, true, true>(a, grid, s) : launch<true, false, true>(a, grid, s);
  return causal ? launch<false, true, true>(a, grid, s) : launch<false, false, true>(a, grid, s);
}

}
```

clip-lora-match_amd/csrc/k_ops.hip:

```cpp
#include "kernels.hpp"

namespace clm {

namespace {

template <bool BF, int NP>
__global__ __launch_bounds__(256) void ln_kernel(LnArgs aa) {
  LnArgs a = aa;
  if (a.m_dev) a.M = __builtin_amdgcn_readfirstlane(*a.m_dev);
  const int lane = threadIdx.x & 63;
  const int row = blockIdx.x * 4 + (threadIdx.x >> 6);
  if (row >= a.M) return;
  const int d = NP * 128;
  float x[NP][2];
  if (a.mode == 0) {
    const float* src = a.src + (int64_t)row * a.lds;
#pragma unroll
    for (int i = 0; i < NP; ++i) {
      const float2 v = *(const float2*)(src + (i * 64 + lane) * 2);
      x[i][0] = v.x; x[i][1] = v.y;
    }
  } else {
    const int src = a.rowmap ? a.rowmap[row] : row;
    const int tokid = a.ids[src];
    const float* tk = a.tok + (int64_t)tokid * d;
    const float* ps = a.pos + (int64_t)(src % a.L) * d;
#pragma unroll
    for (int i = 0; i < NP; ++i) {
      const int e = (i * 64 + lane) * 2;
      const float2 t = *(const float2*)(tk + e);
      const float2 p = *(const float2*)(ps + e);
      x[i][0] = t.x + p.x; x[i][1] = t.y + p.y;
    }
  }
  auto ln = [&](const float* g, const float* b) {
    float s = 0.f;
#pragma unroll
    for (int i = 0; i < NP; ++i) s += x[i][0] + x[i][1];
    const float mean = wave_sum(s) / d;
    float v = 0.f;
#pragma unroll
    for (int i = 0; i < NP; ++i) {
      const float d0 = x[i][0] - mean, d1 = x[i][1] - mean;
      v += d0 * d0 + d1 * d1;
    }
    const float rstd = 1.0f / sqrtf(wave_sum(v) / d + a.eps);
#pragma unroll
    for (int i = 0; i < NP; ++i) {
      const int e = (i * 64 + lane) * 2;
      const float2 gg = *(const float2*)(g + e);
      const float2 bb = *(const float2*)(b + e);
      x[i][0] = (x[i][0] - mean) * rstd * gg.x + bb.x;
      x[i][1] = (x[i][1] - mean) * rstd * gg.y + bb.y;
    }
  };
  auto store_h = [&]() {
    float* h = a.hf + (int64_t)row * a.ldh;
#pragma unroll
    for (int i = 0; i < NP; ++i) *(float2*)(h + (i * 64 + lane) * 2) = make_float2(x[i][0], x[i][1]);
  };
  if (a.g2) {
    ln(a.g1, a.b1);
    store_h();
    ln(a.g2, a.b2);
  } else {
    if (a.mode == 1) store_h();
    ln(a.g1, a.b1);
  }
  u16* y = a.y + (int64_t)row * a.ldy;
#pragma unroll
  for (int i = 0; i < NP; ++i) *(uint32_t*)(y + (i * 64 + lane) * 2) = pack2<BF>(x[i][0], x[i][1]);

}

template <bool BF, int NQ, int R = 2>
__device__ __forceinline__ void ln4_body(const LnArgs& aa, int bid) {
  LnArgs a = aa;
  if (a.m_dev) a.M = __builtin_amdgcn_readfirstlane(*a.m_dev);
  static_assert(R % 2 == 0, "rows per wave come in pairs");
  const int lane = threadIdx.x & 63;
  const int row0 = (bid * 4 + (threadIdx.x >> 6)) * R;
  if (row0 >= a.M) return;
  constexpr int d = NQ * 256;
  float4 x[R][NQ];
#pragma unroll
  for (int r = 0; r < R; ++r) {
    const int row = min(row0 + r, a.M - 1);
    if (a.mode == 0) {
      const float* src = a.src + (int64_t)row * a.lds;
#pragma unroll
      for (int i = 0; i < NQ; ++i) x[r][i] = *(const float4*)(src + (i * 64 + lane) * 4);
    } else {
      const int src = a.rowmap ? a.rowmap[row] : row;
      const int tokid = a.ids[src];
      const float* tk = a.tok + (int64_t)tokid * d;
      const float* ps = a.pos + (int64_t)(src % a.L) * d;
#pragma unroll
      for (int i = 0; i < NQ; ++i) {
        const int e = (i * 64 + lane) * 4;
        const float4 t = *(const float4*)(tk + e), p = *(const float4*)(ps + e);
        x[r][i] = make_float4(t.x + p.x, t.y + p.y, t.z + p.z, t.w + p.w);
      }
    }
  }
  auto ln = [&](const float* g, const float* b) {
    float4 gg[NQ], bb[NQ];
#pragma unroll
    for (int i = 0; i < NQ; ++i) {
      gg[i] = *(const float4*)(g + (i * 64 + lane) * 4);
      bb[i] = *(const float4*)(b + (i * 64 + lane) * 4);
    }
#pragma unroll
    for (int r = 0; r < R; ++r) {
      float s = 0.f;
#pragma unroll
      for (int i = 0; i < NQ; ++i) s += (x[r][i].x + x[r][i].y) + (x[r][i].z + x[r][i].w);
      const float mean = wave_sum(s) / d;
      float v = 0.f;
#pragma unroll
      for (int i = 0; i < NQ; ++i) {
        const float d0 = x[r][i].x - mean, d1 = x[r][i].y - mean, d2 = x[r][i].z - mean, d3 = x[r][i].w - mean;
        v += (d0 * d0 + d1 * d1) + (d2 * d2 + d3 * d3);
      }
      const float rstd = 1.0f / sqrtf(wave_sum(v) / d + a.eps);
#pragma unroll
      for (int i = 0; i < NQ; ++i) {
        x[r][i].x = (x[r][i].x - mean) * rstd * gg[i].x + bb[i].x;
        x[r][i].y = (x[r][i].y - mean) * rstd * gg[i].y + bb[i].y;
        x[r][i].z = (x[r][i].z - mean) * rstd * gg[i].z + bb[i].z;
        x[r][i].w = (x[r][i].w - mean) * rstd * gg[i].w + bb[i].w;
      }
    }
  };
  auto store_h = [&]() {
#pragma unroll
    for (int r = 0; r < R; ++r) {
      if (row0 + r >= a.M) break;
      float* h = a.hf + (int64_t)(row0 + r) * a.ldh;
#pragma unroll
      for (int i = 0; i < NQ; ++i) *(float4*)(h + (i * 64 + lane) * 4) = x[r][i];
    }
  };
  if (a.g2) {
    ln(a.g1, a.b1);
    store_h();
    ln(a.g2, a.b2);
  } else {
    if (a.mode == 1) store_h();
    ln(a.g1, a.b1);
  }
  if (row0 + R - 1 < a.M && (a.ldy % 8) == 0) {
    const bool odd = lane & 1;
#pragma unroll
    for (int r = 0; r < R; r += 2) {
      u16* y0 = a.y + (int64_t)(row0 + r) * a.ldy;
#pragma unroll
      for (int i = 0; i < NQ; ++i) {
        const u32x2 p0{pack2<BF>(x[r][i].x, x[r][i].y), pack2<BF>(x[r][i].z, x[r][i].w)};
        const u32x2 p1{pack2<BF>(x[r + 1][i].x, x[r + 1][i].y), pack2<BF>(x[r + 1][i].z, x[r + 1][i].w)};
        const u32x2 snd = odd ? p0 : p1;
        const u32x2 rcv{(uint32_t)__builtin_amdgcn_update_dpp(0, (int)snd.x, 0xB1, 0xF, 0xF, false),
                        (uint32_t)__builtin_amdgcn_update_dpp(0, (int)snd.y, 0xB1, 0xF, 0xF, false)};
        const int e = (i * 64 + (lane & ~1)) * 4;
        if (!odd) *(u32x4*)(y0 + e) = u32x4{p0.x, p0.y, rcv.x, rcv.y};
        else *(u32x4*)(y0 + a.ldy + e) = u32x4{rcv.x, rcv.y, p1.x, p1.y};
      }
    }
    return;
  }
#pragma unroll
  for (int r = 0; r < R; ++r) {
    if (row0 + r >= a.M) break;
    u16* y = a.y + (int64_t)(row0 + r) * a.ldy;
#pragma unroll
    for (int i = 0; i < NQ; ++i)
      *(u32x2*)(y + (i * 64 + lane) * 4) = u32x2{pack2<BF>(x[r][i].x, x[r][i].y), pack2<BF>(x[r][i].z, x[r][i].w)};
  }
}

template <bool BF, int NQ, int R = 2>
__global__ __launch_bounds__(256) void ln4_kernel(LnArgs a) {
  ln4_body<BF, NQ, R>(a, blockIdx.x);
}

template <bool BF>
hipError_t ln_dispatch(const LnArgs& a, hipStream_t s) {
  dim3 grid((a.M + 3) / 4), block(256);
  dim3 grid2((a.M + 7) / 8);
  switch (a.d) {
    case 128: ln_kernel<BF, 1><<<grid, block, 0, s>>>(a); break;
    case 256: ln4_kernel<BF, 1><<<grid2, block, 0, s>>>(a); break;
    case 512: ln4_kernel<BF, 2><<<grid2, block, 0, s>>>(a); break;
    case 768: ln4_kernel<BF, 3><<<grid2, block, 0, s>>>(a); break;
    case 1024: ln4_kernel<BF, 4><<<grid2, block, 0, s>>>(a); break;
    default: return hipErrorInvalidValue;
  }
  return hipGetLastError();
}

template <bool BF>
__global__ __launch_bounds__(256) void patchify_fast_kernel(const void* pix, int layout, int B, int S, int p,
                                                            const float* lut, u16* P, int Kp) {
  __shared__ float slut[3 * 256];
  for (int i = threadIdx.x; i < 3 * 256; i += blockDim.x) slut[i] = lut[i];
  __syncthreads();
  const int G = S / p, runs = p / 8, pp = p * p;
  const int64_t total = (int64_t)B * G * G * p * runs;
  for (int64_t w = blockIdx.x * (int64_t)blockDim.x + threadIdx.x; w < total;
       w += (int64_t)gridDim.x * blockDim.x) {
    const int run = (int)(w % runs);
    int64_t q = w / runs;
    const int ky = (int)(q % p);
    const int64_t r = q / p;
    const int b = (int)(r / (G * G));
    const int pi = (int)(r - (int64_t)b * G * G);
    const int py = pi / G, px = pi - py * G;
    const int yy = py * p + ky, xx = px * p + run * 8;
    float v[3][8];
    if (layout == 0) {
      const uint8_t* src = (const uint8_t*)pix + (((int64_t)b * S + yy) * S + xx) * 3;
      const uint2 w0 = *(const uint2*)src, w1 = *(const uint2*)(src + 8), w2 = *(const uint2*)(src + 16);
      const uint32_t d[6] = {w0.x, w0.y, w1.x, w1.y, w2.x, w2.y};
#pragma unroll
      for (int e = 0; e < 24; ++e) {
        const uint32_t u = (d[e >> 2] >> ((e & 3) * 8)) & 0xffu;
        v[e % 3][e / 3] = slut[(e % 3) * 256 + u];
      }
    } else {
#pragma unroll
      for (int c = 0; c < 3; ++c) {
        const float* src = (const float*)pix + (((int64_t)b * 3 + c) * S + yy) * S + xx;
        const float4 a0 = *(const float4*)src, a1 = *(const float4*)(src + 4);
        v[c][0] = a0.x; v[c][1] = a0.y; v[c][2] = a0.z; v[c][3] = a0.w;
        v[c][4] = a1.x; v[c][5] = a1.y; v[c][6] = a1.z; v[c][7] = a1.w;
      }
    }
    u16* dst = P + r * Kp + ky * p + run * 8;
#pragma unroll
    for (int c = 0; c < 3; ++c) {
      uint4 o;
      o.x = pack2<BF>(v[c][0], v[c][1]); o.y = pack2<BF>(v[c][2], v[c][3]);
      o.z = pack2<BF>(v[c][4], v[c][5]); o.w = pack2<BF>(v[c][6], v[c][7]);
      *(uint4*)(dst + c * pp) = o;
    }
  }
}

__global__ void pad_cols_kernel(u16* P, int64_t rows, int k0, int Kp) {
  const int w = Kp - k0;
  for (int64_t i = blockIdx.x * (int64_t)blockDim.x + threadIdx.x; i < rows * w; i += (int64_t)gridDim.x * blockDim.x)
    P[(i / w) * Kp + k0 + (i % w)] = 0;
}

template <bool BF>
__global__ __launch_bounds__(256) void patchify_kernel(const void* pix, int layout, int B, int S, int p,
                                                       int C, const float* lut, u16* P, int Kp) {
  const int G = S / p;
  const int64_t rows = (int64_t)B * G * G;
  const int chunks = Kp / 8;
  const int64_t total = rows * chunks;
  const int pp = p * p, kreal = C * pp;
  for (int64_t w = blockIdx.x * (int64_t)blockDim.x + threadIdx.x; w < total;
       w += (int64_t)gridDim.x * blockDim.x) {
    const int64_t r = w / chunks;
    const int kc = (int)(w - r * chunks);
    const int b = (int)(r / (G * G));
    const int pi = (int)(r - (int64_t)b * G * G);
    const int py = pi / G, px = pi - py * G;
    float v[8];
#pragma unroll
    for (int e = 0; e < 8; ++e) {
      const int k = kc * 8 + e;
      float val = 0.f;
      if (k < kreal) {
        const int c = k / pp, rem = k - c * pp;
        const int ky = rem / p, kx = rem - ky * p;
        const int yy = py * p + ky, xx = px * p + kx;
        if (layout == 0) {
          const uint8_t u = ((const uint8_t*)pix)[(((int64_t)b * S + yy) * S + xx) * C + c];
          val = lut[c * 256 + u];
        } else {
          val = ((const float*)pix)[(((int64_t)b * C + c) * S + yy) * S + xx];
        }
      }
      v[e] = val;
    }
    uint4 o;
    o.x = pack2<BF>(v[0], v[1]); o.y = pack2<BF>(v[2], v[3]);
    o.z = pack2<BF>(v[4], v[5]); o.w = pack2<BF>(v[6], v[7]);
    *(uint4*)(P + r * Kp + kc * 8) = o;
  }
}

__global__ void write_cls_kernel(float* h, int64_t ldh, int B, int T, int d, const float* cls,
                                 const float* pos) {
  const int b = blockIdx.x;
  for (int e = threadIdx.x; e < d; e += blockDim.x) h[(int64_t)b * T * ldh + e] = cls[e] + pos[e];
}


__device__ __forceinline__ int pooled_row(const int32_t* ids, int b, int T, int eos, int lane) {
  if (!ids) return 0;
  const int32_t* id = ids + (int64_t)b * T;
  int best = INT_MAX, bestv = INT_MIN;
  for (int t = lane; t < T; t += 64) {
    const int v = id[t];
    if (eos == 2) { if (v > bestv) { bestv = v; best = t; } }
    else if (v == eos && t < best) best = t;
  }
  if (eos == 2) {
    for (int o = 32; o > 0; o >>= 1) {
      const int ov = __shfl_xor(bestv, o, 64), ob = __shfl_xor(best, o, 64);
      if (ov > bestv || (ov == bestv && ob < best)) { bestv = ov; best = ob; }
    }
  } else {
    for (int o = 32; o > 0; o >>= 1) best = min(best, __shfl_xor(best, o, 64));
  }
  return best == INT_MAX ? 0 : best;
}

__global__ __launch_bounds__(64) void gather_pooled_kernel(const float* h, int64_t ldh, const u16* O, int64_t ldo,
                                                           int T, int d, const int32_t* ids, int eos, float* hc,
                                                           u16* Oc, int64_t ldoc, const int* offs) {
  const int b = blockIdx.x, lane = threadIdx.x;
  const int64_t row = offs ? (int64_t)offs[b + 1] - 1 : (int64_t)b * T + pooled_row(ids, b, T, eos, lane);
  for (int e = lane * 4; e < d; e += 256) {
    *(float4*)(hc + (int64_t)b * d + e) = *(const float4*)(h + row * ldh + e);
    *(u32x2*)(Oc + (int64_t)b * ldoc + e) = *(const u32x2*)(O + row * ldo + e);
  }
}

constexpr int PRB = 8, PP = 16;
__global__ __launch_bounds__(64 * PP) void pool_project_kernel(const float* h, int64_t ldh, int B, int T, int d,
                                                               const int32_t* ids, int eos, const float* g,
                                                               const float* bt, float eps, const float* projT, int D,
                                                               float* tmp, const int* offs) {
#pragma clang fp contract(off)
  extern __shared__ __attribute__((aligned(16))) float sm[];
  float* y = sm;
  float* part_sum = sm + d * PRB;
  const int tid = threadIdx.x, lane = tid & 63, wid = tid >> 6;
  const int b0 = blockIdx.x * PRB;
  for (int rr = wid; rr < PRB; rr += PP) {
    const int b = b0 + rr;
    if (b >= B) {
      for (int e = lane; e < d; e += 64) y[e * PRB + rr] = 0.f;
      continue;
    }
    const int64_t prow = offs ? (int64_t)offs[b + 1] - 1 : (int64_t)b * T + pooled_row(ids, b, T, eos, lane);
    const float* x = h + prow * ldh;
    float s = 0.f;
    for (int e = lane; e < d; e += 64) s += x[e];
    const float mean = wave_sum(s) / d;
    float v = 0.f;
    for (int e = lane; e < d; e += 64) { const float t = x[e] - mean; v = fmaf(t, t, v); }
    const float rstd = 1.0f / sqrtf(wave_sum(v) / d + eps);
    for (int e = lane; e < d; e += 64) y[e * PRB + rr] = fmaf((x[e] - mean) * rstd, g[e], bt[e]);
  }
  __syncthreads();
  const int c = lane, part = wid;
  const int j = blockIdx.y * 64 + c;
  const int i0 = part * (d / PP), i1 = i0 + d / PP;
  float acc[PRB];
#pragma unroll
  for (int r = 0; r < PRB; ++r) acc[r] = 0.f;
  if (j < D) {
#pragma unroll 8
    for (int i = i0; i < i1; ++i) {
      const float w = projT[(int64_t)i * D + j];
      const float4 ya = *(const float4*)(y + i * PRB), yb = *(const float4*)(y + i * PRB + 4);
      acc[0] = fmaf(ya.x, w, acc[0]); acc[1] = fmaf(ya.y, w, acc[1]);
      acc[2] = fmaf(ya.z, w, acc[2]); acc[3] = fmaf(ya.w, w, acc[3]);
      acc[4] = fmaf(yb.x, w, acc[4]); acc[5] = fmaf(yb.y, w, acc[5]);
      acc[6] = fmaf(yb.z, w, acc[6]); acc[7] = fmaf(yb.w, w, acc[7]);
    }
  }
#pragma unroll
  for (int r = 0; r < PRB; ++r) part_sum[(part * PRB + r) * 64 + c] = acc[r];
  __syncthreads();
  if (wid < PRB && j < D) {
    const int r = wid, b = b0 + r;
    if (b < B) {
      float t = part_sum[r * 64 + c];
#pragma unroll
      for (int q = 1; q < PP; ++q) t += part_sum[(q * PRB + r) * 64 + c];
      tmp[(int64_t)b * D + j] = t;
    }
  }
}

__global__ __launch_bounds__(256) void text_lens_kernel(const int32_t* ids, int B, int L, int eos, int* lens) {
  const int b = blockIdx.x * 4 + (threadIdx.x >> 6);
  if (b >= B) return;
  const int p = pooled_row(ids, b, L, eos, threadIdx.x & 63);
  if ((threadIdx.x & 63) == 0) lens[b] = p + 1;
}

constexpr int PLAN_MAX_B = 4096;
__global__ __launch_bounds__(256) void text_plan_kernel(int B, int L, const int* lens, int* offs, int* tiles,
                                                        int* counts) {
  __shared__ int s_off[PLAN_MAX_B + 1];
  __shared__ int s_next[PLAN_MAX_B];
  __shared__ int s_part[256];
  const int tid = threadIdx.x;
  const int C = (B + 255) / 256;
  const int b0 = min(tid * C, B), b1 = min(b0 + C, B);
  int sum = 0;
  for (int b = b0; b < b1; ++b) { s_off[b] = sum; sum += lens[b]; }
  s_part[tid] = sum;
  __syncthreads();
  if (tid < 64) {
    const int v0 = s_part[tid * 4], v1 = s_part[tid * 4 + 1], v2 = s_part[tid * 4 + 2], v3 = s_part[tid * 4 + 3];
    const int own = v0 + v1 + v2 + v3;
    int t = own;
    for (int o = 1; o < 64; o <<= 1) {
      const int y = __shfl_up(t, o, 64);
      if (tid >= o) t += y;
    }
    const int ex = t - own;
    s_part[tid * 4] = ex;
    s_part[tid * 4 + 1] = ex + v0;
    s_part[tid * 4 + 2] = ex + v0 + v1;
    s_part[tid * 4 + 3] = ex + v0 + v1 + v2;
    if (tid == 63) {
      s_off[B] = t;
      counts[0] = t;
    }
  }
  __syncthreads();
  for (int b = b0; b < b1; ++b) s_off[b] += s_part[tid];
  __syncthreads();
  for (int b = tid; b < B; b += 256) {
    int lo = b + 1, hi = B;
    const int lim = s_off[b] + 256;
    while (lo < hi) {
      const int mid = (lo + hi + 1) >> 1;
      if (s_off[mid] <= lim) lo = mid; else hi = mid - 1;
    }
    s_next[b] = lo;
  }
  __syncthreads();
  if (tid == 0) {
    int nt = 0;
    for (int first = 0; first < B; first = s_next[first]) tiles[nt++] = first | ((s_next[first] - first) << 16);
    counts[1] = nt;
  }
  for (int b = tid; b <= B; b += 256) offs[b] = s_off[b];
}

constexpr int ROWMAP_CAPS = 16;
__global__ __launch_bounds__(256) void text_rowmap_kernel(int B, int L, const int* offs, int* rowmap) {
  __shared__ int s_o[ROWMAP_CAPS + 1];
  const int b0 = blockIdx.x * ROWMAP_CAPS, nb = min(ROWMAP_CAPS, B - b0);
  if (threadIdx.x <= nb) s_o[threadIdx.x] = offs[b0 + threadIdx.x];
  __syncthreads();
  const int o0 = s_o[0], n = s_o[nb] - o0;
  for (int p = threadIdx.x; p < n; p += 256) {
    const int r = o0 + p;
    int lo = 0, hi = nb - 1;
    while (lo < hi) {
      const int mid = (lo + hi + 1) >> 1;
      if (s_o[mid] <= r) lo = mid; else hi = mid - 1;
    }
    rowmap[r] = (b0 + lo) * L + (r - s_o[lo]);
  }
}

__global__ __launch_bounds__(256) void finish_rows_kernel(const float* tmp, int B, int D, void* out, int out_dtype,
                                                          int normalize) {
#pragma clang fp contract(off)
  const int lane = threadIdx.x & 63;
  const int b = blockIdx.x * 4 + (threadIdx.x >> 6);
  if (b >= B) return;
  const float* r = tmp + (int64_t)b * D;
  float s = 0.f;
  for (int e = lane; e < D; e += 64) s = fmaf(r[e], r[e], s);
  const float nrm = normalize ? sqrtf(wave_sum(s)) : 1.f;
  for (int e = lane; e < D; e += 64) {
    const float o = normalize ? r[e] / nrm : r[e];
    if (out_dtype == 0) ((float*)out)[(int64_t)b * D + e] = o;
    else ((u16*)out)[(int64_t)b * D + e] = f32_to_f16(o);
  }
}

__global__ __launch_bounds__(256) void rows_to_f16_kernel(const void* src, int src_dtype, int64_t n, int dim,
                                                          u16* dst, float* inv_norm, int norm_src) {
  const int lane = threadIdx.x & 63;
  const int64_t row = (int64_t)blockIdx.x * 4 + (threadIdx.x >> 6);
  if (row >= n) return;
  auto load = [&](int e) {
    return src_dtype == 0 ? ((const float*)src)[row * dim + e] : f16_to_f32(((const u16*)src)[row * dim + e]);
  };
  float scale = 1.f;
  if (norm_src == 2) {
    float s0 = 0.f;
    for (int e = lane; e < dim; e += 64) {
      const float v = load(e);
      s0 += v * v;
    }
    scale = 1.0f / sqrtf(wave_sum(s0));
  }
  float s = 0.f;
  for (int e = lane; e < dim; e += 64) {
    const float v = load(e) * scale;
    const u16 hv = f32_to_f16(v);
    dst[row * dim + e] = hv;
    const float r = norm_src == 1 ? v : f16_to_f32(hv);
    s += r * r;
  }
  s = wave_sum(s);
  if (lane == 0) inv_norm[row] = 1.0f / sqrtf(s);
}

__global__ __launch_bounds__(256) void sample_rows_kernel(const u16* rows, const float* inv, int64_t n, int dim,
                                                          int64_t S, u16* out_rows, float* out_inv) {
  const int64_t sidx = blockIdx.x;
  const int64_t src = sidx * n / S;
  const uint4* a = (const uint4*)(rows + src * dim);
  uint4* b = (uint4*)(out_rows + sidx * dim);
  for (int e = threadIdx.x; e < dim / 8; e += blockDim.x) b[e] = a[e];
  if (threadIdx.x == 0) out_inv[sidx] = inv[src];
}

__global__ __launch_bounds__(256) void l2n_kernel(float* rows, int64_t n, int dim) {
  const int lane = threadIdx.x & 63;
  const int64_t row = (int64_t)blockIdx.x * 4 + (threadIdx.x >> 6);
  if (row >= n) return;
  float* r = rows + row * dim;
  float s = 0.f;
  for (int e = lane; e < dim; e += 64) s += r[e] * r[e];
  const float nrm = sqrtf(wave_sum(s));
  for (int e = lane; e < dim; e += 64) r[e] = r[e] / nrm;
}

__global__ __launch_bounds__(256) void fuse_rows_kernel(const float* a, float wa, const float* b, float wb,
                                                         int64_t n, int dim, float* out) {
  const int lane = threadIdx.x & 63;
  const int64_t row = (int64_t)blockIdx.x * 4 + (threadIdx.x >> 6);
  if (row >= n) return;
  const float* ra = a + row * dim;
  const float* rb = b ? b + row * dim : nullptr;
  float* ro = out + row * dim;
  float s = 0.f;
  for (int e = lane; e < dim; e += 64) {
    const float v = rb ? __fadd_rn(__fmul_rn(wa, ra[e]), __fmul_rn(wb, rb[e])) : ra[e];
    s += v * v;
  }
  const float nrm = sqrtf(wave_sum(s));
  for (int e = lane; e < dim; e += 64) {
    const float v = rb ? __fadd_rn(__fmul_rn(wa, ra[e]), __fmul_rn(wb, rb[e])) : ra[e];
    ro[e] = v / nrm;
  }
}

__global__ __launch_bounds__(256) void f32_to_f16_kernel(const float* src, int64_t total, u16* dst) {
  for (int64_t i = blockIdx.x * (int64_t)blockDim.x + threadIdx.x; i < total;
       i += (int64_t)gridDim.x * blockDim.x)
    dst[i] = f32_to_f16(src[i]);
}

}

hipError_t layernorm(bool bf16, const LnArgs& a, hipStream_t s) {
  if (a.M <= 0) return hipSuccess;
  return bf16 ? ln_dispatch<true>(a, s) : ln_dispatch<false>(a, s);
}

hipError_t patchify(bool bf16, const void* pix, int layout, int B, int S, int p, int C, const float* lut,
                    u16* P, int Kp, hipStream_t s) {
  if (B <= 0) return hipSuccess;
  if (Kp % 8) return hipErrorInvalidValue;
  const int G = S / p;
  if (C == 3 && p % 8 == 0 && (S * 3) % 8 == 0) {
    const int64_t total = (int64_t)B * G * G * p * (p / 8);
    const int blocks = (int)std::min<int64_t>((total + 255) / 256, 256 * 32);
    if (bf16) patchify_fast_kernel<true><<<blocks, 256, 0, s>>>(pix, layout, B, S, p, lut, P, Kp);
    else patchify_fast_kernel<false><<<blocks, 256, 0, s>>>(pix, layout, B, S, p, lut, P, Kp);
    if (Kp > 3 * p * p) {
      const int64_t rows = (int64_t)B * G * G;
      pad_cols_kernel<<<(int)std::min<int64_t>((rows * (Kp - 3 * p * p) + 255) / 256, 4096), 256, 0, s>>>(
          P, rows, 3 * p * p, Kp);
    }
    return hipGetLastError();
  }
  const int64_t total = (int64_t)B * G * G * (Kp / 8);
  const int blocks = (int)std::min<int64_t>((total + 255) / 256, 256 * 16);
  if (bf16) patchify_kernel<true><<<blocks, 256, 0, s>>>(pix, layout, B, S, p, C, lut, P, Kp);
  else patchify_kernel<false><<<blocks, 256, 0, s>>>(pix, layout, B, S, p, C, lut, P, Kp);
  return hipGetLastError();
}

hipError_t write_cls(float* h, int64_t ldh, int B, int T, int d, const float* cls, const float* pos,
                     hipStream_t s) {
  if (B <= 0) return hipSuccess;
  write_cls_kernel<<<B, 256, 0, s>>>(h, ldh, B, T, d, cls, pos);
  return hipGetLastError();
}

hipError_t gather_pooled(const float* h, int64_t ldh, const u16* O, int64_t ldo, int B, int T, int d,
                         const int32_t* ids, int eos, float* hc, u16* Oc, int64_t ldoc, hipStream_t s,
                         const int* offs) {
  if (B <= 0) return hipSuccess;
  if ((d % 4) || (ldh % 4) || (ldo % 4) || (ldoc % 4)) return hipErrorInvalidValue;
  gather_pooled_kernel<<<B, 64, 0, s>>>(h, ldh, O, ldo, T, d, ids, eos, hc, Oc, ldoc, offs);
  return hipGetLastError();
}

hipError_t pool_project(const float* h, int64_t ldh, int B, int T, int d, const int32_t* ids, int eos,
                        const float* g, const float* bta, float eps, const float* projT, int D, float* tmp, void* out,
                        int out_dtype, int normalize, hipStream_t s, const int* offs) {
  if (B <= 0) return hipSuccess;
  if (d % PP) return hipErrorInvalidValue;
  const size_t sm = (size_t)(d * PRB + PP * PRB * 64) * sizeof(float);
  dim3 grid((B + PRB - 1) / PRB, (D + 63) / 64);
  pool_project_kernel<<<grid, 64 * PP, sm, s>>>(h, ldh, B, T, d, ids, eos, g, bta, eps, projT, D, tmp, offs);
  finish_rows_kernel<<<(B + 3) / 4, 256, 0, s>>>(tmp, B, D, out, out_dtype, normalize);
  return hipGetLastError();
}

hipError_t text_plan(const int32_t* ids, int B, int L, int eos, int* lens, int* offs, int* rowmap, int* tiles,
                     int* counts, hipStream_t s) {
  if (B <= 0) return hipSuccess;
  if (L < 1 || L > 256) return hipErrorInvalidValue;
  if (B > PLAN_MAX_B) return hipErrorInvalidValue;
  text_lens_kernel<<<(B + 3) / 4, 256, 0, s>>>(ids, B, L, eos, lens);
  text_plan_kernel<<<1, 256, 0, s>>>(B, L, lens, offs, tiles, counts);
  text_rowmap_kernel<<<(B + ROWMAP_CAPS - 1) / ROWMAP_CAPS, 256, 0, s>>>(B, L, offs, rowmap);
  return hipGetLastError();
}

hipError_t rows_to_f16(const void* src, int src_dtype, int64_t n, int dim, u16* dst, float* inv_norm,
                       hipStream_t s, int norm_src) {
  if (n <= 0) return hipSuccess;
  rows_to_f16_kernel<<<(unsigned)((n + 3) / 4), 256, 0, s>>>(src, src_dtype, n, dim, dst, inv_norm, norm_src);
  return hipGetLastError();
}

hipError_t sample_rows(const u16* rows, const float* inv, int64_t n, int dim, int64_t S, u16* out_rows,
                       float* out_inv, hipStream_t s) {
  if (S <= 0) return hipSuccess;
  if (dim % 8) return hipErrorInvalidValue;
  sample_rows_kernel<<<(unsigned)S, 64, 0, s>>>(rows, inv, n, dim, S, out_rows, out_inv);
  return hipGetLastError();
}

hipError_t l2_normalize_rows(float* rows, int64_t n, int dim, hipStream_t s) {
  if (n <= 0) return hipSuccess;
  l2n_kernel<<<(unsigned)((n + 3) / 4), 256, 0, s>>>(rows, n, dim);
  return hipGetLastError();
}

hipError_t fuse_rows(const float* a, float wa, const float* b, float wb, int64_t n, int dim, float* out,
                     hipStream_t s) {
  if (n <= 0) return hipSuccess;
  fuse_rows_kernel<<<(unsigned)((n + 3) / 4), 256, 0, s>>>(a, wa, b, wb, n, dim, out);
  return hipGetLastError();
}

hipError_t f32_to_f16_rows(const float* src, int64_t n, int dim, u16* dst, hipStream_t s) {
  const int64_t total = n * dim;
  if (total <= 0) return hipSuccess;
  const int blocks = (int)std::min<int64_t>((total + 255) / 256, 4096);
  f32_to_f16_kernel<<<blocks, 256, 0, s>>>(src, total, dst);
  return hipGetLastError();
}

}
```

clip-lora-match_amd/csrc/kernels.hpp:

```cpp
#pragma once
#include "clm_common.hpp"

namespace clm {

enum Epi {
  EPI_STORE = 0,
  EPI_GELU = 1,
  EPI_RESID = 2,
  EPI_PATCH = 3,
  EPI_SCORE = 4,
  EPI_FILTER = 5,
  EPI_RANK = 6
};
constexpr bool epi_stores16(int e) { return e == EPI_STORE || e == EPI_GELU; }
constexpr bool epi_gelu(int e) { return e == EPI_GELU; }

struct GemmArgs {
  const u16* A; int64_t lda;
  const u16* W; int64_t ldw;
  int M, N, K;
  void* out; int64_t ldo;
  const float* bias;
  const float* aux; int64_t aux_ld; int group;
  const float* rscale; const float* cscale;
  const float* theta; int64_t theta_ld; int* cnt; float* cand_s; int64_t* cand_i; int cap; int64_t base;
  const unsigned* cbound;
  unsigned* above; float rank_margin;
  int m_fastest;
  int ksplit; int64_t split_stride;
  int out16;
  const int* m_dev;
  int debug;
};

hipError_t gemm(bool bf16, int epi, const GemmArgs& g, hipStream_t s);
hipError_t gemm_splitk_resid(bool bf16, const GemmArgs& g, int slices, float* ws, hipStream_t s);
inline size_t gemm_splitk_ws_bytes(int M, int N, int slices) { return (size_t)slices * M * N * 4; }
constexpr int GEMM_CFG_SPLITK = 2;
constexpr int GEMM_CFG_SKINNY = 12;
hipError_t gemm_cfg(bool bf16, int epi, int config, const GemmArgs& g, hipStream_t s);
int gemm_num_configs();
void gemm_set_concurrent(bool on);

struct LnArgs {
  int mode;
  const float* src; int64_t lds;
  const int32_t* ids; const float* tok; const float* pos; int L;
  float* hf; int64_t ldh;
  const float* g1; const float* b1;
  const float* g2; const float* b2;
  u16* y; int64_t ldy;
  int M, d; float eps;
  const int* m_dev; const int* rowmap;
};
hipError_t layernorm(bool bf16, const LnArgs& a, hipStream_t s);

struct ResizeDesc {
  int64_t src_off;
  int64_t tmp_off;
  int32_t W, r0, rows, kh, kv, coef_off;
};
hipError_t resize_crop(const uint8_t* src, const ResizeDesc* desc, int n, int S, int max_rows,
                       const int32_t* coef, uint8_t* tmp, uint8_t* out, hipStream_t s);

hipError_t synth_images(uint64_t seed, int64_t row0, int n, int S, uint8_t* out, hipStream_t s);

hipError_t patchify(bool bf16, const void* pix, int layout, int B, int S, int p, int C,
                    const float* lut , u16* P, int Kp, hipStream_t s);

hipError_t write_cls(float* h, int64_t ldh, int B, int T, int d, const float* cls,
                     const float* pos, hipStream_t s);

hipError_t gather_pooled(const float* h, int64_t ldh, const u16* O, int64_t ldo, int B, int T, int d,
                         const int32_t* ids, int eos, float* hc, u16* Oc, int64_t ldoc, hipStream_t s,
                         const int* offs = nullptr);
hipError_t pool_project(const float* h, int64_t ldh, int B, int T, int d, const int32_t* ids,
                        int eos, const float* g, const float* bta, float eps, const float* projT,
                        int D, float* tmp, void* out, int out_dtype, int normalize, hipStream_t s,
                        const int* offs = nullptr);
hipError_t text_plan(const int32_t* ids, int B, int L, int eos, int* lens, int* offs, int* rowmap, int* tiles,
                     int* counts, hipStream_t s);

bool attention_folds_log2e(bool bf16, bool causal, int T);
hipError_t attention(bool bf16, bool causal, const u16* qkv, int64_t ldq, u16* out, int64_t ldo,
                     int B, int T, int H, int d, hipStream_t s, bool q_log2e = false);
bool gemm_attn_supported(int T, int H, int d, int K);
hipError_t gemm_attn(bool bf16, bool causal, const u16* X, int64_t ldx, const u16* W, int64_t ldw, const float* bias,
                     u16* out, int64_t ldo, int B, int T, int H, int d, int K, hipStream_t s);
hipError_t gemm_attn_varlen(bool bf16, bool causal, const u16* X, int64_t ldx, const u16* W, int64_t ldw,
                            const float* bias, u16* out, int64_t ldo, int B, int L, int H, int d, int K,
                            const int* lens, const int* offs, const int* tiles, const int* counts, hipStream_t s);
struct AttnProblem {
  const u16* X; int64_t ldx; const u16* W; int64_t ldw; const float* bias; u16* out; int64_t ldo;
  int B, T, H, d, K;
  const int *lens, *offs, *tiles, *counts;
};

hipError_t rows_to_f16(const void* src, int src_dtype, int64_t n, int dim, u16* dst,
                       float* inv_norm, hipStream_t s, int norm_src);
hipError_t topk_rows(const float* scores, int64_t lds, int64_t nq, int64_t C, int k,
                     int64_t base, float* out_s, int64_t* out_i, int64_t ldo, hipStream_t s);
size_t topk_any_ws_bytes(int64_t nq, int k);
hipError_t topk_any(const float* scores, int64_t lds, const int64_t* idx, int64_t ldi, int64_t nq, int64_t C, int k,
                    int64_t base, float* out_s, int64_t* out_i, int64_t ldo, void* ws, hipStream_t s);
hipError_t count_ge(const float* scores, int64_t lds, int64_t nq, int64_t C, const float* th, int* cnt, hipStream_t s);
hipError_t count_ge16(const u16* scores, int64_t lds, int64_t nq, int64_t C, const float* th, int* cnt, hipStream_t s);
hipError_t kth_thresholds16(const u16* scores, int64_t lds, int64_t nq, int64_t C, int k, float margin, float* th,
                            hipStream_t s);
hipError_t topk_merge(const float* in_s, const int64_t* in_i, int64_t nq, int parts, int k_in,
                      int k, float* out_s, int64_t* out_i, hipStream_t s);
hipError_t max_index(const int64_t* idx, int64_t n, int64_t* out, hipStream_t s);
hipError_t l2_normalize_rows(float* rows, int64_t n, int dim, hipStream_t s);
hipError_t fuse_rows(const float* a, float wa, const float* b, float wb, int64_t n, int dim, float* out,
                     hipStream_t s);
hipError_t sample_rows(const u16* rows, const float* inv, int64_t n, int dim, int64_t S, u16* out_rows,
                       float* out_inv, hipStream_t s);
hipError_t f32_to_f16_rows(const float* src, int64_t n, int dim, u16* dst, hipStream_t s);
hipError_t f16_to_f32_rows(const u16* src, int64_t n, int dim, float* dst, hipStream_t s);

hipError_t query_norms(const float* q, int64_t nq, int dim, double* qn, hipStream_t s);
hipError_t exact_scores(const float* q, const double* qn, int64_t nq, const void* rows, bool rows_f16, int64_t rn,
                        int dim, float* out, int64_t ldo, hipStream_t s);
hipError_t rescore_select(const float* cand_s, const int64_t* cand_i, const int* cnt, int cap, const float* q,
                          const double* qn, int dim, const void* rows, bool rows_f16, int64_t offset, float margin,
                          int64_t nq, int k, float* out_s, int64_t* out_i, hipStream_t s);
constexpr int RESCORE_WIDE_CHUNK = 4096;
hipError_t rescore_wide(const int64_t* cand_i, const int* cnt, int64_t cap, const float* q, const double* qn, int dim,
                        const void* rows, bool rows_f16, int64_t offset, int64_t nq, int k, float* part_s,
                        int64_t* part_i, hipStream_t s);
hipError_t gather_rows(const void* src, int64_t src_stride, const int64_t* idx, int64_t n, int64_t row_bytes,
                       void* dst, int64_t dst_stride, bool scatter, hipStream_t s);
hipError_t filter_thresholds(const float* ts, int64_t ld, int64_t nq, int k, float margin, float* th, hipStream_t s);
hipError_t kth_thresholds(const float* scores, int64_t lds, int64_t nq, int64_t C, int k, float margin, float* th,
                          hipStream_t s);
hipError_t value_bounds(const float* v, int64_t n, unsigned* keys, hipStream_t s);
struct Scan16Args {
  const u16* rows; const float* inv; int64_t N; int dim;
  const u16* q16; const float* qinv; int nq;
  float* out; int64_t ldo;
  float* cmax; int64_t nchunk;
  float* wtop; int64_t ldw;
};
hipError_t scan16(const Scan16Args& a, hipStream_t s);
void scan16_shape(int dim, int* nw, int* depth);
int scan16_grid(int64_t nchunk, int nw, int cus);
int64_t scan16_waves(int64_t nchunk, int dim);
hipError_t collect_ge(const float* scores, int ldq, int nq, int64_t C, const float* th, int* cnt, int cap, float* cs,
                      int64_t* ci, int64_t base, hipStream_t s);

__host__ __device__ inline bool rank_ahead(float s, int64_t idx, float t, int64_t g) {
  const bool sn = s != s, tn = t != t;
  if (sn || tn) return sn && (!tn || idx < g);
  return s > t || (s == t && idx < g);
}
hipError_t target_scores(const float* q, const double* qn, int64_t nq, int dim, const void* rows, bool rows_f16,
                         int64_t offset, const int64_t* target, float* t, hipStream_t s);
hipError_t rank_rescore(const int64_t* band, const int* cnt, int64_t cap, const unsigned* above32, const float* q,
                        const double* qn, int dim, const void* rows, bool rows_f16, int64_t offset, const float* t,
                        const int64_t* g, int64_t nq, int* plan, int64_t* out, hipStream_t s);
hipError_t count_rank(const float* scores, int64_t lds, int64_t nq, int64_t C, int64_t base, const float* t,
                      const int64_t* g, int64_t* above, hipStream_t s);
hipError_t rank_from_above(const int64_t* above, int64_t nq, int64_t* rank, hipStream_t s);

__host__ __device__ inline unsigned float_key(float f) {
  const unsigned b = __builtin_bit_cast(unsigned, f);
  return (b & 0x80000000u) ? ~b : (b | 0x80000000u);
}
__host__ __device__ inline float key_float(unsigned k) {
  return __builtin_bit_cast(float, (k & 0x80000000u) ? (k & 0x7FFFFFFFu) : ~k);
}

}
```

Measured before the change: 51500 image+text pairs/s.

## Compute last-layer attention only for pooled query rows and fold gather into split-K LN

```diff
diff --git a/clip-lora-match_amd/csrc/capi.cpp b/clip-lora-match_amd/csrc/capi.cpp
--- a/clip-lora-match_amd/csrc/capi.cpp
+++ b/clip-lora-match_amd/csrc/capi.cpp
@@ -111,6 +111,7 @@
   float* pooled = nullptr;
   float* hc = nullptr;
   u16* Oc = nullptr;
+  int* prow = nullptr;
   int *vl_lens = nullptr, *vl_offs = nullptr, *vl_rowmap = nullptr, *vl_tiles = nullptr, *vl_counts = nullptr;
   int64_t ldx = 0, ldo = 0, ldm = 0;
 };
@@ -419,6 +420,7 @@
   if ((r = c->dalloc(&T.pooled, (size_t)B * d.proj_dim))) return r;
   if ((r = c->dalloc(&T.hc, (size_t)B * T.d))) return r;
   if ((r = c->dalloc(&T.Oc, (size_t)B * T.ldo))) return r;
+  if ((r = c->dalloc(&T.prow, (size_t)B))) return r;
   if (!T.vision) {
     if ((r = c->dalloc(&T.vl_lens, (size_t)B))) return r;
     if ((r = c->dalloc(&T.vl_offs, (size_t)2 * B + 1))) return r;
@@ -516,6 +518,8 @@
   return v == 1 && !(g_gemm_debug & 16) && gemm_attn_supported(T, H, d, K);
 }
 
+bool prune_attention() { return prune_last_layer() && !(g_gemm_debug & 64); }
+
 struct LayerRun {
   Tower* T;
   int B, S;
@@ -544,6 +548,11 @@
   return 2.0 * R.Mx * 3 * T.d * T.layers[l].kl_qkv + 4.0 * T.H * R.attn_pairs * 64;
 }
 
+bool pooled_queries(const LayerRun& R, int l) {
+  const Tower& T = *R.T;
+  return prune_attention() && l + 1 == T.L && (R.vl || fused_attention(R.S, T.H, T.d, T.layers[l].kl_qkv));
+}
+
 int attn_step(clm_ctx* c, const LayerRun& R, int l, hipStream_t st) {
   Tower& T = *R.T;
   LayerW& Lw = T.layers[l];
@@ -551,7 +560,13 @@
   GemmArgs g{};
   g.A = T.X; g.lda = T.ldx; g.M = R.B * R.S; g.N = 3 * T.d; g.K = Lw.kl_qkv; g.out = T.QKV; g.ldo = 3 * T.d;
   g.W = Lw.w_qkv; g.ldw = Lw.k_qkv; g.bias = Lw.b_qkv;
-  if (R.vl) {
+  if (pooled_queries(R, l)) {
+    PROF(CLM_PROF_GEMM, 2.0 * R.Mx * 2 * T.d * g.K + 2.0 * R.B * T.d * g.K + 4.0 * T.H * R.Mx * 64);
+    AttnProblem p{g.A, g.lda, g.W, g.ldw, g.bias, T.Oc, T.ldo, R.B, R.S, T.H, T.d, g.K, nullptr, nullptr, nullptr,
+                  nullptr, R.ids, c->desc.eos_token_id, T.prow};
+    if (R.vl) { p.lens = T.vl_lens; p.offs = T.vl_offs; p.tiles = T.vl_tiles; p.counts = T.vl_counts; }
+    KCHK(gemm_attn_pooled(bf, R.causal, p, st));
+  } else if (R.vl) {
     PROF(CLM_PROF_GEMM, attn_flops(R, l));
     KCHK(gemm_attn_varlen(bf, R.causal, g.A, g.lda, g.W, g.ldw, g.bias, T.O, T.ldo, R.B, R.S, T.H, T.d, g.K,
                           T.vl_lens, T.vl_offs, T.vl_tiles, T.vl_counts, st));
@@ -566,13 +581,17 @@
   return CLM_OK;
 }
 
-int pooled_resid(clm_ctx* c, const LayerRun& R, GemmArgs& g, hipStream_t st) {
+int pooled_slices(const LayerRun& R, const GemmArgs& g) {
   const int nk = g.K / 64;
-  int slices = 1;
   for (int sl = nk / 4; sl >= 2; --sl)
-    if (nk % sl == 0 && gemm_splitk_ws_bytes(1, g.N, sl) <= (size_t)R.S * 3 * R.T->d * 2) { slices = sl; break; }
+    if (nk % sl == 0 && gemm_splitk_ws_bytes(1, g.N, sl) <= (size_t)R.S * 3 * R.T->d * 2) return sl;
+  return 1;
+}
+int pooled_resid(clm_ctx* c, const LayerRun& R, GemmArgs& g, hipStream_t st, const float* src = nullptr,
+                 int64_t lds = 0, const int* row_of = nullptr) {
+  const int slices = pooled_slices(R, g);
   PROF(CLM_PROF_GEMM, 2.0 * g.M * g.N * g.K);
-  if (slices > 1) KCHK(gemm_splitk_resid(R.bf, g, slices, (float*)R.T->QKV, st));
+  if (slices > 1) KCHK(gemm_splitk_resid(R.bf, g, slices, (float*)R.T->QKV, st, src, lds, row_of));
   else KCHK(gemm_cfg(R.bf, EPI_RESID, GEMM_CFG_SPLITK, g, st));
   return CLM_OK;
 }
@@ -618,26 +637,42 @@
   int64_t M = (int64_t)R.B * R.S;
   float* h = T.h;
   u16* O = T.O;
+  const bool pooled_q = pooled && pooled_queries(R, l);
+  bool fold_gather = false;
   if (pooled) {
-    { PROF(CLM_PROF_OTHER, (double)R.B * T.d * 6.0);
-      KCHK(gather_pooled(T.h, T.d, T.O, T.ldo, R.B, R.S, T.d, R.ids, c->desc.eos_token_id, T.hc, T.Oc, T.ldo, st,
-                         R.vl ? T.vl_offs : nullptr)); }
     M = R.B;
     h = T.hc;
     O = T.Oc;
     *pooled_rows = true;
   }
   PostOps p = post_ops(c, R, l, M, h, O, pooled);
+  if (pooled) {
+    fold_gather = pooled_q && pooled_slices(R, p.out) > 1;
+    if (!fold_gather) {
+      PROF(CLM_PROF_OTHER, (double)R.B * T.d * (pooled_q ? 4.0 : 6.0));
+      KCHK(gather_pooled(T.h, T.d, pooled_q ? nullptr : T.O, T.ldo, R.B, R.S, T.d, R.ids, c->desc.eos_token_id, T.hc,
+                         T.Oc, T.ldo, st, R.vl ? T.vl_offs : nullptr));
+    }
+  }
   const int* mdev = pooled ? nullptr : R.mdev;
   if (Lw.r_out) { PROF(CLM_PROF_GEMM, 2.0 * p.rows * RPAD * T.d);
     KCHK(lora_down_gemm(bf, O, T.ldo, (int)M, T.d, Lw.a_out, mdev, st)); }
-  if (pooled) {
-    int r = pooled_resid(c, R, p.out, st);
-    if (r) return r;
+  if (fold_gather && layernorm_sums_slices(T.d)) {
+    const int slices = pooled_slices(R, p.out);
+    { PROF(CLM_PROF_GEMM, 2.0 * p.out.M * p.out.N * p.out.K);
+      KCHK(gemm_splitk_partials(bf, p.out, slices, (float*)T.QKV, st)); }
+    p.ln2.mode = 2; p.ln2.src = T.h; p.ln2.lds = T.d; p.ln2.row_of = T.prow;
+    p.ln2.ws = (const float*)T.QKV; p.ln2.slices = slices; p.ln2.sbias = p.out.bias;
+    { PROF(CLM_PROF_LN, p.rows * T.d * 6.0); KCHK(layernorm(bf, p.ln2, st)); }
   } else {
-    PROF(CLM_PROF_GEMM, 2.0 * p.rows * p.out.N * p.out.K); KCHK(gemm(bf, EPI_RESID, p.out, st));
-  }
-  { PROF(CLM_PROF_LN, p.rows * T.d * 6.0); KCHK(layernorm(bf, p.ln2, st)); }
+    if (pooled) {
+      int r = fold_gather ? pooled_resid(c, R, p.out, st, T.h, T.d, T.prow) : pooled_resid(c, R, p.out, st);
+      if (r) return r;
+    } else {
+      PROF(CLM_PROF_GEMM, 2.0 * p.rows * p.out.N * p.out.K); KCHK(gemm(bf, EPI_RESID, p.out, st));
+    }
+    { PROF(CLM_PROF_LN, p.rows * T.d * 6.0); KCHK(layernorm(bf, p.ln2, st)); }
+  }
   if (Lw.r_fc1) { PROF(CLM_PROF_GEMM, 2.0 * p.rows * RPAD * T.d);
     KCHK(lora_down_gemm(bf, T.X, T.ldx, (int)M, T.d, Lw.a_fc1, mdev, st)); }
   { PROF(CLM_PROF_GEMM, 2.0 * p.rows * p.fc1.N * p.fc1.K);
@@ -679,6 +714,7 @@
   T.pooled += (int64_t)b0 * proj_dim;
   T.hc += (int64_t)b0 * T.d;
   T.Oc += (int64_t)b0 * T.ldo;
+  T.prow += b0;
   if (T.vl_lens) {
     T.vl_lens += b0; T.vl_tiles += b0; T.vl_offs += 2 * b0; T.vl_counts += 2 * b0; T.vl_rowmap += r0;
   }
diff --git a/clip-lora-match_amd/csrc/clm_common.hpp b/clip-lora-match_amd/csrc/clm_common.hpp
--- a/clip-lora-match_amd/csrc/clm_common.hpp
+++ b/clip-lora-match_amd/csrc/clm_common.hpp
@@ -1,5 +1,6 @@
 #pragma once
 #include <hip/hip_runtime.h>
+#include <limits.h>
 #include <stdint.h>
 
 typedef uint16_t u16;
@@ -78,6 +79,26 @@
 __device__ __forceinline__ float group16_sum(float v) { return row16_reduce<false>(v); }
 __device__ __forceinline__ float group16_max(float v) { return row16_reduce<true>(v); }
 
+__device__ __forceinline__ int pooled_row(const int32_t* ids, int b, int T, int eos, int lane) {
+  if (!ids) return 0;
+  const int32_t* id = ids + (int64_t)b * T;
+  int best = INT_MAX, bestv = INT_MIN;
+  for (int t = lane; t < T; t += 64) {
+    const int v = id[t];
+    if (eos == 2) { if (v > bestv) { bestv = v; best = t; } }
+    else if (v == eos && t < best) best = t;
+  }
+  if (eos == 2) {
+    for (int o = 32; o > 0; o >>= 1) {
+      const int ov = __shfl_xor(bestv, o, 64), ob = __shfl_xor(best, o, 64);
+      if (ov > bestv || (ov == bestv && ob < best)) { bestv = ov; best = ob; }
+    }
+  } else {
+    for (int o = 32; o > 0; o >>= 1) best = min(best, __shfl_xor(best, o, 64));
+  }
+  return best == INT_MAX ? 0 : best;
+}
+
 __device__ __forceinline__ uint32_t f16_down(float v) {
   const _Float16 h = (_Float16)v;
   uint32_t b = __builtin_bit_cast(uint16_t, h);
diff --git a/clip-lora-match_amd/csrc/k_gemm.hip b/clip-lora-match_amd/csrc/k_gemm.hip
--- a/clip-lora-match_amd/csrc/k_gemm.hip
+++ b/clip-lora-match_amd/csrc/k_gemm.hip
@@ -320,7 +320,8 @@
 
 namespace {
 __global__ __launch_bounds__(256) void splitk_resid_kernel(const float* ws, int slices, int M, int N, const float* bias,
-                                                          float* out, int64_t ldo) {
+                                                          float* out, int64_t ldo, const float* src, int64_t lds,
+                                                          const int* row_of) {
   const int n4 = N / 4;
   const int64_t i = (int64_t)blockIdx.x * 256 + threadIdx.x;
   if (i >= (int64_t)M * n4) return;
@@ -333,23 +334,32 @@
   }
   const float4 b = bias ? *(const float4*)(bias + n) : make_float4(0.f, 0.f, 0.f, 0.f);
   float4* o = (float4*)(out + (int64_t)m * ldo + n);
-  float4 h = *o;
+  float4 h = src ? *(const float4*)(src + (int64_t)row_of[m] * lds + n) : *o;
   h.x = h.x + (acc.x + b.x); h.y = h.y + (acc.y + b.y); h.z = h.z + (acc.z + b.z); h.w = h.w + (acc.w + b.w);
   *o = h;
 }
 }
 
-hipError_t gemm_splitk_resid(bool bf16, const GemmArgs& g, int slices, float* ws, hipStream_t s) {
+hipError_t gemm_splitk_resid(bool bf16, const GemmArgs& g, int slices, float* ws, hipStream_t s, const float* src,
+                             int64_t lds, const int* row_of) {
   if (g.M <= 0 || g.N <= 0) return hipSuccess;
   if (slices < 1 || g.K <= 0 || g.K % (BK * slices) || (g.N % 4) || (g.ldo % 4) || !ws) return hipErrorInvalidValue;
+  if (src && (!row_of || (lds % 4))) return hipErrorInvalidValue;
+  hipError_t e = gemm_splitk_partials(bf16, g, slices, ws, s);
+  if (e != hipSuccess) return e;
+  const int64_t n = (int64_t)g.M * (g.N / 4);
+  splitk_resid_kernel<<<(unsigned)((n + 255) / 256), 256, 0, s>>>(ws, slices, g.M, g.N, g.bias, (float*)g.out, g.ldo, src, lds,
+                                                                 row_of);
+  return hipGetLastError();
+}
+
+hipError_t gemm_splitk_partials(bool bf16, const GemmArgs& g, int slices, float* ws, hipStream_t s) {
+  if (g.M <= 0 || g.N <= 0) return hipSuccess;
+  if (slices < 1 || g.K <= 0 || g.K % (BK * slices) || !ws) return hipErrorInvalidValue;
   GemmArgs p = g;
   p.out = ws; p.ldo = g.N; p.bias = nullptr; p.rscale = nullptr; p.cscale = nullptr;
   p.ksplit = slices; p.split_stride = (int64_t)g.M * g.N;
-  hipError_t e = gemm_cfg(bf16, EPI_SCORE, GEMM_CFG_SPLITK, p, s);
-  if (e != hipSuccess) return e;
-  const int64_t n = (int64_t)g.M * (g.N / 4);
-  splitk_resid_kernel<<<(unsigned)((n + 255) / 256), 256, 0, s>>>(ws, slices, g.M, g.N, g.bias, (float*)g.out, g.ldo);
-  return hipGetLastError();
+  return gemm_cfg(bf16, EPI_SCORE, GEMM_CFG_SPLITK, p, s);
 }
 
 void gemm_set_concurrent(bool on) { g_concurrent = on; }
diff --git a/clip-lora-match_amd/csrc/k_gemm_attn.hip b/clip-lora-match_amd/csrc/k_gemm_attn.hip
--- a/clip-lora-match_amd/csrc/k_gemm_attn.hip
+++ b/clip-lora-match_amd/csrc/k_gemm_attn.hip
@@ -15,6 +15,8 @@
 constexpr int FA_SEC = FA_BM * 128;
 static_assert(3 * FA_SEC <= FA_LDS, "q/k/v staging must fit in the ring's LDS");
 static_assert(FA_BM % (8 * FA_NW) == 0 && FA_BN % (8 * FA_NW) == 0, "rows split evenly over waves");
+constexpr int FA_TNP = 4, FA_QP = 8;
+constexpr int FA_LDS_POOL = FA_LDS + FA_BM * 4;
 
 __device__ __forceinline__ int swz_s(int row, int chunk) { return chunk ^ (row & 7); }
 
@@ -38,9 +40,81 @@
   u16* out; int64_t ldo;
   int B, T, H, d, K, G;
   const int* lens; const int* offs; const int* tiles; const int* counts;
+  const int32_t* ids; int eos; int* prow;
 };
 
-template <bool BF, bool CAUSAL, bool VL>
+template <bool BF, bool CAUSAL>
+__device__ __forceinline__ void attn_unit(const uint8_t* sQ, const uint8_t* sK, const uint8_t* sV, int qrow, int qi,
+                                          int q0, int T, int r0, int lane, u16* op) {
+  constexpr float L2E = 1.4426950408889634f;
+  const int g = lane >> 4;
+  const int ntiles = (T + 63) / 64;
+  u32x4 qa[2];
+#pragma unroll
+  for (int kk = 0; kk < 2; ++kk) qa[kk] = *(const u32x4*)(sQ + qrow * 128 + swz_s(qrow, kk * 4 + g) * 16);
+  const int nkt = CAUSAL ? min((q0 + 15) / 64 + 1, ntiles) : ntiles;
+  f32x4 sc[2][4];
+  float tmax = -INFINITY;
+#pragma unroll
+  for (int kt = 0; kt < 2; ++kt) {
+    if (kt >= nkt) break;
+#pragma unroll
+    for (int nb = 0; nb < 4; ++nb) {
+      sc[kt][nb] = f32x4{0.f, 0.f, 0.f, 0.f};
+      const int krow = min(r0 + kt * 64 + nb * 16 + (lane & 15), FA_BM - 1);
+#pragma unroll
+      for (int kk = 0; kk < 2; ++kk) {
+        const int c = kk * 4 + g;
+        sc[kt][nb] = mfma16<BF>(*(const u32x4*)(sK + krow * 128 + swz_s(krow, c) * 16), qa[kk], sc[kt][nb]);
+      }
+#pragma unroll
+      for (int j = 0; j < 4; ++j) {
+        const int kj = kt * 64 + nb * 16 + 4 * g + j;
+        if (!(kj < T && (!CAUSAL || kj <= qi))) sc[kt][nb][j] = -INFINITY;
+        tmax = fmaxf(tmax, sc[kt][nb][j]);
+      }
+    }
+  }
+  tmax = cross_rows_reduce<true>(tmax);
+  const float m2 = tmax * L2E;
+  float rs = 0.f;
+  f32x4 o[4];
+#pragma unroll
+  for (int nb = 0; nb < 4; ++nb) o[nb] = f32x4{0.f, 0.f, 0.f, 0.f};
+#pragma unroll
+  for (int kt = 0; kt < 2; ++kt) {
+    if (kt >= nkt) break;
+    u32x4 pb[2];
+#pragma unroll
+    for (int nb = 0; nb < 4; ++nb)
+#pragma unroll
+      for (int j = 0; j < 4; ++j) {
+        const float p = __builtin_amdgcn_exp2f(fmaf(sc[kt][nb][j], L2E, -m2));
+        sc[kt][nb][j] = p;
+        rs += p;
+      }
+#pragma unroll
+    for (int kk = 0; kk < 2; ++kk) {
+      const f32x4 lo = sc[kt][2 * kk], hi = sc[kt][2 * kk + 1];
+      pb[kk] = u32x4{pack2<BF>(lo[0], lo[1]), pack2<BF>(lo[2], lo[3]), pack2<BF>(hi[0], hi[1]),
+                     pack2<BF>(hi[2], hi[3])};
+    }
+#pragma unroll
+    for (int kk = 0; kk < 2; ++kk)
+#pragma unroll
+      for (int nb = 0; nb < 4; ++nb)
+        o[nb] = mfma16<BF>(v_frag_rows(sV, r0 + kt * 64 + kk * 32, nb, lane), pb[kk], o[nb]);
+  }
+  rs = cross_rows_reduce<false>(rs);
+  if (op) {
+    const float inv = 1.0f / rs;
+#pragma unroll
+    for (int nb = 0; nb < 4; ++nb)
+      *(u32x2*)(op + nb * 16) = u32x2{pack2<BF>(o[nb][0] * inv, o[nb][1] * inv), pack2<BF>(o[nb][2] * inv, o[nb][3] * inv)};
+  }
+}
+
+template <bool BF, bool CAUSAL, bool VL, bool POOL>
 __device__ __forceinline__ void gemm_attn_body(const FaArgs& a, int bid, int nwg) {
   extern __shared__ __attribute__((aligned(16))) uint8_t smem[];
   const int tid = threadIdx.x, lane = tid & 63, g = lane >> 4;
@@ -64,6 +138,30 @@
     M = (int64_t)a.B * a.T;
   }
   const int h = t % a.H;
+  constexpr int TN = POOL ? FA_TNP : FA_TN, WCOLS = TN * 16, C0 = POOL ? 64 : 0;
+  int* s_prow = (int*)(smem + FA_LDS);
+  int nqp = 0, qrow[FA_QP];
+  if constexpr (POOL) {
+    if constexpr (VL) {
+      for (int i = tid; i < nseq; i += FA_NW * 64) s_prow[i] = a.offs[s0 + i + 1] - 1 - (int)m0;
+    } else if (a.ids) {
+      for (int i = wid; i < nseq; i += FA_NW) {
+        const int p = pooled_row(a.ids, s0 + i, a.T, a.eos, lane);
+        if (lane == 0) s_prow[i] = i * a.T + p;
+      }
+    } else {
+      for (int i = tid; i < nseq; i += FA_NW * 64) s_prow[i] = i * a.T;
+    }
+    __syncthreads();
+    if (h == 0 && a.prow)
+      for (int i = tid; i < nseq; i += FA_NW * 64) a.prow[s0 + i] = (int)m0 + s_prow[i];
+    nqp = max(0, ((nseq + 15) / 16 - (wid >> 2) + 1) / 2);
+#pragma unroll
+    for (int i = 0; i < FA_QP; ++i) {
+      const int p = ((wid >> 2) + 2 * i) * 16 + (lane & 15);
+      qrow[i] = p < nseq ? s_prow[p] : 0;
+    }
+  }
   const int nk = (a.K + BK - 1) / BK;
   const bool half_last = (a.K % BK) != 0;
 
@@ -94,17 +192,24 @@
   };
 
   const int wm = wid / FA_WN, wn = wid % FA_WN;
-  float4 bv[FA_TN];
-#pragma unroll
-  for (int nb = 0; nb < FA_TN; ++nb) {
-    const int col = wn * (FA_BN / FA_WN) + nb * 16 + 4 * g;
+  float4 bv[TN];
+#pragma unroll
+  for (int nb = 0; nb < TN; ++nb) {
+    const int col = C0 + wn * WCOLS + nb * 16 + 4 * g;
     bv[nb] = a.bias ? *(const float4*)(a.bias + (col >> 6) * a.d + h * 64 + (col & 63)) : make_float4(0.f, 0.f, 0.f, 0.f);
   }
-  f32x4 acc[FA_TM][FA_TN];
+  f32x4 acc[FA_TM][TN];
 #pragma unroll
   for (int i = 0; i < FA_TM; ++i)
 #pragma unroll
-    for (int j = 0; j < FA_TN; ++j) acc[i][j] = f32x4{0.f, 0.f, 0.f, 0.f};
+    for (int j = 0; j < TN; ++j) acc[i][j] = f32x4{0.f, 0.f, 0.f, 0.f};
+  float4 bq = make_float4(0.f, 0.f, 0.f, 0.f);
+  f32x4 qacc[POOL ? FA_QP : 1];
+  if constexpr (POOL) {
+    if (a.bias) bq = *(const float4*)(a.bias + h * 64 + (wid & 3) * 16 + 4 * g);
+#pragma unroll
+    for (int i = 0; i < FA_QP; ++i) qacc[i] = f32x4{0.f, 0.f, 0.f, 0.f};
+  }
 
   stage(0, 0);
   for (int s = 0; s < nk; ++s) {
@@ -117,48 +222,84 @@
     for (int kk = 0; kk < 2; ++kk) {
       if (kk == 1 && half_last && s == nk - 1) break;
       const int c = kk * 4 + g;
-      u32x4 af[FA_TM], bw[FA_TN];
+      u32x4 af[FA_TM], bw[TN];
 #pragma unroll
       for (int mb = 0; mb < FA_TM; ++mb) {
         const int row = wm * (FA_BM / FA_WM) + mb * 16 + (lane & 15);
         af[mb] = *(const u32x4*)(sa + row * 128 + swz(row, c) * 16);
       }
 #pragma unroll
-      for (int nb = 0; nb < FA_TN; ++nb) {
-        const int row = wn * (FA_BN / FA_WN) + nb * 16 + (lane & 15);
+      for (int nb = 0; nb < TN; ++nb) {
+        const int row = C0 + wn * WCOLS + nb * 16 + (lane & 15);
         bw[nb] = *(const u32x4*)(sb + row * 128 + swz(row, c) * 16);
       }
 #pragma unroll
       for (int mb = 0; mb < FA_TM; ++mb)
 #pragma unroll
-        for (int nb = 0; nb < FA_TN; ++nb) acc[mb][nb] = mfma16<BF>(bw[nb], af[mb], acc[mb][nb]);
+        for (int nb = 0; nb < TN; ++nb) acc[mb][nb] = mfma16<BF>(bw[nb], af[mb], acc[mb][nb]);
+      if constexpr (POOL) {
+        if (nqp > 0) {
+          const int wrow = (wid & 3) * 16 + (lane & 15);
+          const u32x4 wq = *(const u32x4*)(sb + wrow * 128 + swz(wrow, c) * 16);
+#pragma unroll
+          for (int i = 0; i < FA_QP; ++i)
+            if (i < nqp)
+              qacc[i] = mfma16<BF>(wq, *(const u32x4*)(sa + qrow[i] * 128 + swz(qrow[i], c) * 16), qacc[i]);
+        }
+      }
     }
   }
 
   lds_barrier();
-  static_assert(FA_TN % 2 == 0, "column blocks are swapped in pairs");
+  static_assert(TN % 2 == 0, "column blocks are swapped in pairs");
 #pragma unroll
   for (int mb = 0; mb < FA_TM; ++mb) {
     const int row = wm * (FA_BM / FA_WM) + mb * 16 + (lane & 15);
 #pragma unroll
-    for (int nb = 0; nb < FA_TN; nb += 2) {
+    for (int nb = 0; nb < TN; nb += 2) {
       const u32x2 p0{pack2<BF>(acc[mb][nb][0] + bv[nb].x, acc[mb][nb][1] + bv[nb].y),
                      pack2<BF>(acc[mb][nb][2] + bv[nb].z, acc[mb][nb][3] + bv[nb].w)};
       const u32x2 p1{pack2<BF>(acc[mb][nb + 1][0] + bv[nb + 1].x, acc[mb][nb + 1][1] + bv[nb + 1].y),
                      pack2<BF>(acc[mb][nb + 1][2] + bv[nb + 1].z, acc[mb][nb + 1][3] + bv[nb + 1].w)};
       const auto rx = __builtin_amdgcn_permlane16_swap(p0.x, p1.x, false, false);
       const auto ry = __builtin_amdgcn_permlane16_swap(p0.y, p1.y, false, false);
-      const int col = wn * (FA_BN / FA_WN) + (nb + (g & 1)) * 16 + (g >> 1) * 8;
+      const int col = C0 + wn * WCOLS + (nb + (g & 1)) * 16 + (g >> 1) * 8;
       const int dim = col & 63;
       *(u32x4*)(smem + (col >> 6) * FA_SEC + row * 128 + (swz_s(row, dim >> 3) << 4)) = u32x4{rx[0], ry[0], rx[1], ry[1]};
     }
   }
+  if constexpr (POOL) {
+#pragma unroll
+    for (int i = 0; i < FA_QP; ++i) {
+      const int p = ((wid >> 2) + 2 * i) * 16 + (lane & 15);
+      if (i < nqp && p < nseq) {
+        const int dim = (wid & 3) * 16 + 4 * g;
+        *(u32x2*)(smem + p * 128 + (swz_s(p, dim >> 3) << 4) + (dim & 7) * 2) =
+            u32x2{pack2<BF>(qacc[i][0] + bq.x, qacc[i][1] + bq.y), pack2<BF>(qacc[i][2] + bq.z, qacc[i][3] + bq.w)};
+      }
+    }
+  }
   lds_barrier();
 
-  constexpr float L2E = 1.4426950408889634f;
   const uint8_t* sQ = smem;
   const uint8_t* sK = smem + FA_SEC;
   const uint8_t* sV = smem + 2 * FA_SEC;
+  if constexpr (POOL) {
+    for (int i = wid; i < nseq; i += FA_NW) {
+      int T, r0;
+      if constexpr (VL) {
+        T = a.lens[s0 + i];
+        r0 = a.offs[s0 + i] - (int)m0;
+      } else {
+        T = a.T;
+        r0 = i * a.T;
+      }
+      const int qi = s_prow[i] - r0;
+      u16* op = (lane & 15) == 0 ? a.out + (int64_t)(s0 + i) * a.ldo + h * 64 + 4 * g : nullptr;
+      attn_unit<BF, CAUSAL>(sQ, sK, sV, i, qi, qi & ~15, T, r0, lane, op);
+    }
+    return;
+  }
   int u = 0, i = 0, qb = 0, nqb = 0, seq_t = 0, seq_r0 = 0;
   auto load_seq = [&]() {
     if constexpr (VL) {
@@ -177,95 +318,30 @@
     const bool mine = (u % FA_NW) == wid;
     if (++qb == nqb && ++i < nseq) load_seq();
     if (!mine) continue;
-    const int ntiles = (T + 63) / 64;
     const int qi = q0 + (lane & 15);
-    u32x4 qa[2];
-    {
-      const int qrow = r0 + min(qi, T - 1);
-#pragma unroll
-      for (int kk = 0; kk < 2; ++kk) qa[kk] = *(const u32x4*)(sQ + qrow * 128 + swz_s(qrow, kk * 4 + g) * 16);
-    }
-    const int nkt = CAUSAL ? min((q0 + 15) / 64 + 1, ntiles) : ntiles;
-    f32x4 sc[2][4];
-    float tmax = -INFINITY;
-#pragma unroll
-    for (int kt = 0; kt < 2; ++kt) {
-      if (kt >= nkt) break;
-#pragma unroll
-      for (int nb = 0; nb < 4; ++nb) {
-        sc[kt][nb] = f32x4{0.f, 0.f, 0.f, 0.f};
-        const int krow = min(r0 + kt * 64 + nb * 16 + (lane & 15), FA_BM - 1);
-#pragma unroll
-        for (int kk = 0; kk < 2; ++kk) {
-          const int c = kk * 4 + g;
-          sc[kt][nb] = mfma16<BF>(*(const u32x4*)(sK + krow * 128 + swz_s(krow, c) * 16), qa[kk], sc[kt][nb]);
-        }
-#pragma unroll
-        for (int j = 0; j < 4; ++j) {
-          const int kj = kt * 64 + nb * 16 + 4 * g + j;
-          if (!(kj < T && (!CAUSAL || kj <= qi))) sc[kt][nb][j] = -INFINITY;
-          tmax = fmaxf(tmax, sc[kt][nb][j]);
-        }
-      }
-    }
-    tmax = cross_rows_reduce<true>(tmax);
-    const float m2 = tmax * L2E;
-    float rs = 0.f;
-    f32x4 o[4];
-#pragma unroll
-    for (int nb = 0; nb < 4; ++nb) o[nb] = f32x4{0.f, 0.f, 0.f, 0.f};
-#pragma unroll
-    for (int kt = 0; kt < 2; ++kt) {
-      if (kt >= nkt) break;
-      u32x4 pb[2];
-#pragma unroll
-      for (int nb = 0; nb < 4; ++nb)
-#pragma unroll
-        for (int j = 0; j < 4; ++j) {
-          const float p = __builtin_amdgcn_exp2f(fmaf(sc[kt][nb][j], L2E, -m2));
-          sc[kt][nb][j] = p;
-          rs += p;
-        }
-#pragma unroll
-      for (int kk = 0; kk < 2; ++kk) {
-        const f32x4 lo = sc[kt][2 * kk], hi = sc[kt][2 * kk + 1];
-        pb[kk] = u32x4{pack2<BF>(lo[0], lo[1]), pack2<BF>(lo[2], lo[3]), pack2<BF>(hi[0], hi[1]),
-                       pack2<BF>(hi[2], hi[3])};
-      }
-#pragma unroll
-      for (int kk = 0; kk < 2; ++kk)
-#pragma unroll
-        for (int nb = 0; nb < 4; ++nb)
-          o[nb] = mfma16<BF>(v_frag_rows(sV, r0 + kt * 64 + kk * 32, nb, lane), pb[kk], o[nb]);
-    }
-    rs = cross_rows_reduce<false>(rs);
-    if (qi < T) {
-      const float inv = 1.0f / rs;
-      u16* op = a.out + (m0 + r0 + qi) * a.ldo + h * 64 + 4 * g;
-#pragma unroll
-      for (int nb = 0; nb < 4; ++nb)
-        *(u32x2*)(op + nb * 16) = u32x2{pack2<BF>(o[nb][0] * inv, o[nb][1] * inv), pack2<BF>(o[nb][2] * inv, o[nb][3] * inv)};
-    }
-  }
-}
-
-template <bool BF, bool CAUSAL, bool VL>
+    u16* op = qi < T ? a.out + (m0 + r0 + qi) * a.ldo + h * 64 + 4 * g : nullptr;
+    attn_unit<BF, CAUSAL>(sQ, sK, sV, r0 + min(qi, T - 1), qi, q0, T, r0, lane, op);
+  }
+}
+
+template <bool BF, bool CAUSAL, bool VL, bool POOL>
 __global__ __launch_bounds__(FA_NW * 64, 2) void gemm_attn_kernel(FaArgs a) {
-  gemm_attn_body<BF, CAUSAL, VL>(a, blockIdx.x, gridDim.x);
-}
-
-template <bool BF, bool CAUSAL, bool VL>
+  gemm_attn_body<BF, CAUSAL, VL, POOL>(a, blockIdx.x, gridDim.x);
+}
+
+template <bool BF, bool CAUSAL, bool VL, bool POOL = false>
 hipError_t launch(const FaArgs& a, int tiles, hipStream_t s) {
-  auto kern = gemm_attn_kernel<BF, CAUSAL, VL>;
+  auto kern = gemm_attn_kernel<BF, CAUSAL, VL, POOL>;
+  constexpr int lds = POOL ? FA_LDS_POOL : FA_LDS;
   static unsigned dev_done = 0;
   int dev = 0;
   (void)hipGetDevice(&dev);
   if (!(__atomic_load_n(&dev_done, __ATOMIC_ACQUIRE) & (1u << (dev & 31)))) {
-    hipError_t e = hipFuncSetAttribute((const void*)kern, hipFuncAttributeMaxDynamicSharedMemorySize, FA_LDS);
+    hipError_t e = hipFuncSetAttribute((const void*)kern, hipFuncAttributeMaxDynamicSharedMemorySize, lds);
     if (e != hipSuccess) return e;
     __atomic_fetch_or(&dev_done, 1u << (dev & 31), __ATOMIC_RELEASE);
   }
-  kern<<<dim3(tiles), dim3(FA_NW * 64), FA_LDS, s>>>(a);
+  kern<<<dim3(tiles), dim3(FA_NW * 64), lds, s>>>(a);
   return hipGetLastError();
 }
 }
@@ -282,6 +358,7 @@
   a = FaArgs{};
   a.X = p.X; a.ldx = p.ldx; a.W = p.W; a.ldw = p.ldw; a.bias = p.bias; a.out = p.out; a.ldo = p.ldo;
   a.B = p.B; a.T = p.T; a.H = p.H; a.d = p.d; a.K = p.K; a.G = FA_BM / p.T;
+  a.ids = p.ids; a.eos = p.eos; a.prow = p.prow;
   const int64_t tiles = (int64_t)((p.B + a.G - 1) / a.G) * p.H;
   if (tiles > 0x7FFFFFFF) return false;
   grid = (int)tiles;
@@ -295,6 +372,7 @@
   a.X = p.X; a.ldx = p.ldx; a.W = p.W; a.ldw = p.ldw; a.bias = p.bias; a.out = p.out; a.ldo = p.ldo;
   a.B = p.B; a.T = p.T; a.H = p.H; a.d = p.d; a.K = p.K; a.G = 0;
   a.lens = p.lens; a.offs = p.offs; a.tiles = p.tiles; a.counts = p.counts;
+  a.prow = p.prow;
   const int64_t max_tiles = std::min<int64_t>(p.B, ((int64_t)p.B * p.T + (256 - p.T)) / (257 - p.T) + 1);
   const int64_t g = max_tiles * p.H;
   if (g > 0x7FFFFFFF) return false;
@@ -326,4 +404,18 @@
   return causal ? launch<false, true, true>(a, grid, s) : launch<false, false, true>(a, grid, s);
 }
 
-}
+hipError_t gemm_attn_pooled(bool bf16, bool causal, const AttnProblem& p, hipStream_t s) {
+  if (p.B <= 0) return hipSuccess;
+  FaArgs a;
+  int grid;
+  if (p.lens) {
+    if (!varlen_args(p, a, grid)) return hipErrorInvalidValue;
+    if (bf16) return causal ? launch<true, true, true, true>(a, grid, s) : launch<true, false, true, true>(a, grid, s);
+    return causal ? launch<false, true, true, true>(a, grid, s) : launch<false, false, true, true>(a, grid, s);
+  }
+  if (!fixed_args(p, a, grid)) return hipErrorInvalidValue;
+  if (bf16) return causal ? launch<true, true, false, true>(a, grid, s) : launch<true, false, false, true>(a, grid, s);
+  return causal ? launch<false, true, false, true>(a, grid, s) : launch<false, false, false, true>(a, grid, s);
+}
+
+}
diff --git a/clip-lora-match_amd/csrc/k_ops.hip b/clip-lora-match_amd/csrc/k_ops.hip
--- a/clip-lora-match_amd/csrc/k_ops.hip
+++ b/clip-lora-match_amd/csrc/k_ops.hip
@@ -90,6 +90,21 @@
       const float* src = a.src + (int64_t)row * a.lds;
 #pragma unroll
       for (int i = 0; i < NQ; ++i) x[r][i] = *(const float4*)(src + (i * 64 + lane) * 4);
+    } else if (a.mode == 2) {
+      const float* src = a.src + (int64_t)(a.row_of ? a.row_of[row] : row) * a.lds;
+      const int64_t stride = (int64_t)a.M * d;
+#pragma unroll
+      for (int i = 0; i < NQ; ++i) {
+        const int e = (i * 64 + lane) * 4;
+        float4 acc = *(const float4*)(a.ws + (int64_t)row * d + e);
+        for (int s = 1; s < a.slices; ++s) {
+          const float4 p = *(const float4*)(a.ws + s * stride + (int64_t)row * d + e);
+          acc.x += p.x; acc.y += p.y; acc.z += p.z; acc.w += p.w;
+        }
+        const float4 b = a.sbias ? *(const float4*)(a.sbias + e) : make_float4(0.f, 0.f, 0.f, 0.f);
+        const float4 h = *(const float4*)(src + e);
+        x[r][i] = make_float4(h.x + (acc.x + b.x), h.y + (acc.y + b.y), h.z + (acc.z + b.z), h.w + (acc.w + b.w));
+      }
     } else {
       const int src = a.rowmap ? a.rowmap[row] : row;
       const int tokid = a.ids[src];
@@ -146,7 +161,7 @@
     store_h();
     ln(a.g2, a.b2);
   } else {
-    if (a.mode == 1) store_h();
+    if (a.mode != 0) store_h();
     ln(a.g1, a.b1);
   }
   if (row0 + R - 1 < a.M && (a.ldy % 8) == 0) {
@@ -299,26 +314,6 @@
 }
 
 
-__device__ __forceinline__ int pooled_row(const int32_t* ids, int b, int T, int eos, int lane) {
-  if (!ids) return 0;
-  const int32_t* id = ids + (int64_t)b * T;
-  int best = INT_MAX, bestv = INT_MIN;
-  for (int t = lane; t < T; t += 64) {
-    const int v = id[t];
-    if (eos == 2) { if (v > bestv) { bestv = v; best = t; } }
-    else if (v == eos && t < best) best = t;
-  }
-  if (eos == 2) {
-    for (int o = 32; o > 0; o >>= 1) {
-      const int ov = __shfl_xor(bestv, o, 64), ob = __shfl_xor(best, o, 64);
-      if (ov > bestv || (ov == bestv && ob < best)) { bestv = ov; best = ob; }
-    }
-  } else {
-    for (int o = 32; o > 0; o >>= 1) best = min(best, __shfl_xor(best, o, 64));
-  }
-  return best == INT_MAX ? 0 : best;
-}
-
 __global__ __launch_bounds__(64) void gather_pooled_kernel(const float* h, int64_t ldh, const u16* O, int64_t ldo,
                                                            int T, int d, const int32_t* ids, int eos, float* hc,
                                                            u16* Oc, int64_t ldoc, const int* offs) {
@@ -326,7 +321,7 @@
   const int64_t row = offs ? (int64_t)offs[b + 1] - 1 : (int64_t)b * T + pooled_row(ids, b, T, eos, lane);
   for (int e = lane * 4; e < d; e += 256) {
     *(float4*)(hc + (int64_t)b * d + e) = *(const float4*)(h + row * ldh + e);
-    *(u32x2*)(Oc + (int64_t)b * ldoc + e) = *(const u32x2*)(O + row * ldo + e);
+    if (O) *(u32x2*)(Oc + (int64_t)b * ldoc + e) = *(const u32x2*)(O + row * ldo + e);
   }
 }
 
@@ -563,6 +558,8 @@
 
 hipError_t layernorm(bool bf16, const LnArgs& a, hipStream_t s) {
   if (a.M <= 0) return hipSuccess;
+  if (a.mode == 2 && (!layernorm_sums_slices(a.d) || !a.ws || a.slices < 1 || a.m_dev || a.g2 || (a.lds % 4)))
+    return hipErrorInvalidValue;
   return bf16 ? ln_dispatch<true>(a, s) : ln_dispatch<false>(a, s);
 }
 
diff --git a/clip-lora-match_amd/csrc/kernels.hpp b/clip-lora-match_amd/csrc/kernels.hpp
--- a/clip-lora-match_amd/csrc/kernels.hpp
+++ b/clip-lora-match_amd/csrc/kernels.hpp
@@ -34,7 +34,9 @@
 };
 
 hipError_t gemm(bool bf16, int epi, const GemmArgs& g, hipStream_t s);
-hipError_t gemm_splitk_resid(bool bf16, const GemmArgs& g, int slices, float* ws, hipStream_t s);
+hipError_t gemm_splitk_resid(bool bf16, const GemmArgs& g, int slices, float* ws, hipStream_t s,
+                             const float* src = nullptr, int64_t lds = 0, const int* row_of = nullptr);
+hipError_t gemm_splitk_partials(bool bf16, const GemmArgs& g, int slices, float* ws, hipStream_t s);
 inline size_t gemm_splitk_ws_bytes(int M, int N, int slices) { return (size_t)slices * M * N * 4; }
 constexpr int GEMM_CFG_SPLITK = 2;
 constexpr int GEMM_CFG_SKINNY = 12;
@@ -52,8 +54,10 @@
   u16* y; int64_t ldy;
   int M, d; float eps;
   const int* m_dev; const int* rowmap;
+  const float* ws; int slices; const float* sbias; const int* row_of;
 };
 hipError_t layernorm(bool bf16, const LnArgs& a, hipStream_t s);
+inline bool layernorm_sums_slices(int d) { return d == 256 || d == 512 || d == 768 || d == 1024; }
 
 struct ResizeDesc {
   int64_t src_off;
@@ -94,7 +98,9 @@
   const u16* X; int64_t ldx; const u16* W; int64_t ldw; const float* bias; u16* out; int64_t ldo;
   int B, T, H, d, K;
   const int *lens, *offs, *tiles, *counts;
+  const int32_t* ids; int eos; int* prow;
 };
+hipError_t gemm_attn_pooled(bool bf16, bool causal, const AttnProblem& p, hipStream_t s);
 
 hipError_t rows_to_f16(const void* src, int src_dtype, int64_t n, int dim, u16* dst,
                        float* inv_norm, hipStream_t s, int norm_src);
```

Measured after the change: 51850 image+text pairs/s (median of 6 runs). No clear change (+0.7%).
